# SYSTRAN/faster-whisper

Hardware: AMD Instinct MI355X
Metric: audio-sec/sec (RTF) large-v3 fp16 beam=5 batch=16 (higher is better)
Workload: dtype f16

## Files before the change

### faster_whisper_amd/_lib.py

```python
import ctypes as C
import os

import numpy as np

_HERE = os.path.dirname(os.path.abspath(__file__))
LIB_PATH = os.environ.get("FWAMD_LIB") or os.path.join(_HERE, "libfwamd.so")

FW_OK = 0
FW_EINVAL = -1
FW_ENODEV = -2
FW_ENOMEM = -3
FW_ERUNTIME = -4
FW_ENOSPC = -5

COMPUTE_FLOAT16 = 0
COMPUTE_INT8_FLOAT16 = 1
FW_DT_F32 = 0
FW_DT_F16 = 1
FW_MAX_ALIGN_HEADS = 64


class FwConfig(C.Structure):
    _fields_ = [
        ("n_mels", C.c_int32), ("n_audio_ctx", C.c_int32), ("d_model", C.c_int32), ("n_heads", C.c_int32),
        ("n_enc_layers", C.c_int32), ("n_dec_layers", C.c_int32), ("n_vocab", C.c_int32),
        ("n_text_ctx", C.c_int32), ("is_multilingual", C.c_int32),
        ("tok_eot", C.c_int32), ("tok_sot", C.c_int32), ("tok_lang_begin", C.c_int32), ("n_langs", C.c_int32),
        ("tok_translate", C.c_int32), ("tok_transcribe", C.c_int32), ("tok_sot_lm", C.c_int32),
        ("tok_sot_prev", C.c_int32), ("tok_no_speech", C.c_int32), ("tok_no_timestamps", C.c_int32),
        ("tok_timestamp_begin", C.c_int32),
        ("n_suppress_begin", C.c_int32), ("suppress_begin", C.c_int32 * 8),
        ("n_align_heads", C.c_int32), ("align_heads", C.c_int32 * (2 * FW_MAX_ALIGN_HEADS)),
    ]


class FwWeight(C.Structure):
    _fields_ = [("name", C.c_char_p), ("data", C.c_void_p), ("dtype", C.c_int32), ("ndim", C.c_int32),
                ("dims", C.c_int64 * 4)]


class FwGenOpts(C.Structure):
    _fields_ = [
        ("beam_size", C.c_int32), ("patience", C.c_float), ("num_hypotheses", C.c_int32),
        ("length_penalty", C.c_float), ("repetition_penalty", C.c_float), ("no_repeat_ngram_size", C.c_int32),
        ("max_length", C.c_int32), ("return_scores", C.c_int32), ("return_no_speech_prob", C.c_int32),
        ("max_initial_timestamp_index", C.c_int32), ("suppress_blank", C.c_int32),
        ("suppress_tokens", C.POINTER(C.c_int32)), ("n_suppress_tokens", C.c_int32),
        ("sampling_topk", C.c_int32), ("sampling_temperature", C.c_float), ("seed", C.c_uint64),
        ("min_new_tokens", C.c_int32),
    ]


class FwVadWeights(C.Structure):
    _fields_ = [
        ("stft_basis", C.c_void_p), ("conv_w", C.c_void_p * 4), ("conv_b", C.c_void_p * 4),
        ("lstm_w", C.c_void_p), ("lstm_r", C.c_void_p), ("lstm_b", C.c_void_p), ("dec_w", C.c_void_p),
        ("dec_b", C.c_float),
    ]


SYMBOLS = [
    "fw_last_error", "fw_abi_version", "fw_device_count",
    "fw_model_create", "fw_model_free", "fw_model_info", "fw_model_blob", "fw_model_create_from_blob_dev",
    "fw_model_set_decode_batch", "fw_model_decode_batch", "fw_model_join_decoder", "fw_model_decode_stats",
    "fw_model_set_merge_wait", "fw_model_set_decode_lanes", "fw_model_run_capacity", "fw_dec_big_min_rows", "fw_dec_big_min_rows_of", "fw_test_knob",
    "fw_test_idle_lead_chunks",
    "fw_pack_blob_size", "fw_pack_blob_copy", "fw_pack_blob_free",
    "fw_logmel", "fw_logmel_full",
    "fw_encode", "fw_encode_pcm", "fw_encode_pcm_dev", "fw_tensor_shape", "fw_tensor_to_host",
    "fw_tensor_from_host", "fw_tensor_free",
    "fw_generate", "fw_detect_language", "fw_align",
    "fw_prof_enable", "fw_prof_reset", "fw_prof_count", "fw_prof_name", "fw_prof_get", "fw_synchronize",
    "fw_dev_alloc", "fw_dev_free", "fw_dev_upload",
    "fw_test_gemm", "fw_test_layernorm", "fw_test_attention", "fw_test_dec_linear", "fw_test_dec_logits", "fw_test_logits_rules",
    "fw_test_dec_self_attn", "fw_test_dec_cross_attn", "fw_test_dec_cross_probs", "fw_test_dec_softmax_pick", "fw_bench_gemm", "fw_bench_dec_linear", "fw_bench_attention",
    "fw_bench_gemm_epi", "fw_bench_dec_linear_epi",
    "fw_test_gemm_ex", "fw_test_cross_kv_frag_index", "fw_test_quant_rows", "fw_test_layernorm_frag",
    "fw_vad_create", "fw_vad_forward", "fw_vad_free", "fw_vad_forward_dev", "fw_vad_forward_audio_dev",
    "fw_flac_info", "fw_flac_decode",
    "fw_resample_filter", "fw_resample_dev", "fw_bench_resample",
]

_lib = None


class FwError(RuntimeError):
    pass


def load():
    global _lib
    if _lib is not None:
        return _lib
    if not os.path.exists(LIB_PATH):
        raise FwError(
            f"{LIB_PATH} not found: build it with `python -c 'import __graft_entry__ as g; g.build()'` "
            "(hipcc --offload-arch=gfx950). faster_whisper_amd has no CPU fallback.")
    lib = C.CDLL(LIB_PATH)
    vp, i32, i64, f32p = C.c_void_p, C.c_int32, C.c_int64, C.POINTER(C.c_float)
    i32p, i64p = C.POINTER(C.c_int32), C.POINTER(C.c_int64)
    lib.fw_last_error.restype = C.c_char_p
    lib.fw_abi_version.restype = i32
    lib.fw_device_count.restype = i32
    lib.fw_model_create.argtypes = [C.POINTER(FwConfig), C.POINTER(FwWeight), i32, i32, i32, i32, i32, C.POINTER(vp)]
    lib.fw_model_free.argtypes = [vp]
    lib.fw_model_free.restype = None
    lib.fw_model_info.argtypes = [vp, C.POINTER(FwConfig), i32p, i32p, i32p, i32p]
    lib.fw_model_blob.argtypes = [vp, C.POINTER(vp), i64p]
    lib.fw_model_create_from_blob_dev.argtypes = [C.POINTER(FwConfig), vp, i64, i32, i32, i32, i32, C.POINTER(vp)]
    lib.fw_model_set_decode_batch.argtypes = [vp, i32]
    lib.fw_model_decode_batch.argtypes = [vp]
    lib.fw_model_decode_batch.restype = i32
    lib.fw_model_run_capacity.argtypes = [vp]
    lib.fw_model_run_capacity.restype = i32
    lib.fw_dec_big_min_rows.restype = i32
    if hasattr(lib, "fw_dec_big_min_rows_of"):
        lib.fw_dec_big_min_rows_of.restype = i32
        lib.fw_dec_big_min_rows_of.argtypes = [i32, i32]
    if hasattr(lib, "fw_flac_info"):
        lib.fw_flac_info.argtypes = [vp, i64, i32p, i32p, i32p, i64p]
        lib.fw_flac_decode.argtypes = [vp, i64, vp, i64, i64p, i32p]
    if hasattr(lib, "fw_test_knob"):
        lib.fw_test_knob.argtypes = [i32, i32]
    if hasattr(lib, "fw_test_idle_lead_chunks"):
        lib.fw_test_idle_lead_chunks.argtypes = [i64, i32, i32, i64, i32]
        lib.fw_test_idle_lead_chunks.restype = i64
    lib.fw_model_join_decoder.argtypes = [vp, vp]
    lib.fw_model_set_merge_wait.argtypes = [vp, i32, i32]
    lib.fw_model_set_decode_lanes.argtypes = [vp, i32]
    lib.fw_model_decode_stats.argtypes = [vp, i64p, i64p, i64p, i32p]
    lib.fw_pack_blob_size.argtypes = [C.POINTER(FwConfig), C.POINTER(FwWeight), i32, i32, i64p, C.POINTER(vp)]
    lib.fw_pack_blob_copy.argtypes = [vp, vp, i64]
    lib.fw_pack_blob_free.argtypes = [vp]
    lib.fw_pack_blob_free.restype = None
    lib.fw_logmel.argtypes = [vp, vp, i64p, i32, vp, i32p]
    lib.fw_logmel_full.argtypes = [vp, vp, i64, vp, i64]
    lib.fw_encode.argtypes = [vp, vp, i32, C.POINTER(vp)]
    lib.fw_encode_pcm.argtypes = [vp, vp, i64p, i32, C.POINTER(vp)]
    lib.fw_encode_pcm_dev.argtypes = [vp, vp, i64p, i32, C.POINTER(vp)]
    lib.fw_tensor_shape.argtypes = [vp, i32p, i32p, i32p]
    lib.fw_tensor_to_host.argtypes = [vp, vp, vp]
    lib.fw_tensor_from_host.argtypes = [vp, vp, i32, C.POINTER(vp)]
    lib.fw_tensor_free.argtypes = [vp]
    lib.fw_tensor_free.restype = None
    lib.fw_generate.argtypes = [vp, vp, i32p, i32p, i32, C.POINTER(FwGenOpts), i32p, i32p, f32p, f32p]
    lib.fw_detect_language.argtypes = [vp, vp, i32, i32p, f32p]
    lib.fw_align.argtypes = [vp, vp, i32p, i32, i32p, i32p, i32p, i32, i32, i32, i32p, i32p, f32p]
    lib.fw_prof_enable.argtypes = [vp, i32]
    lib.fw_prof_enable.restype = None
    lib.fw_prof_reset.argtypes = [vp]
    lib.fw_prof_reset.restype = None
    lib.fw_prof_count.restype = i32
    lib.fw_prof_name.argtypes = [i32]
    lib.fw_prof_name.restype = C.c_char_p
    lib.fw_prof_get.argtypes = [vp, i32, C.POINTER(C.c_double), i64p, C.POINTER(C.c_double), C.POINTER(C.c_double)]
    lib.fw_synchronize.argtypes = [vp]
    lib.fw_dev_alloc.argtypes = [vp, i64, C.POINTER(vp)]
    lib.fw_dev_free.argtypes = [vp, vp]
    lib.fw_dev_upload.argtypes = [vp, vp, vp, i64]
    lib.fw_test_gemm.argtypes = [vp, vp, vp, vp, vp, i32, i32, i32, i32, i32, vp]
    lib.fw_test_dec_linear.argtypes = [vp, vp, vp, vp, vp, vp, vp, i32, i32, i32, i32, i32, vp, vp]
    lib.fw_test_dec_logits.argtypes = [vp, vp, i32, vp]
    lib.fw_test_logits_rules.argtypes = [vp, vp, i32, vp, i32, vp, C.POINTER(FwGenOpts), i32, vp, vp]
    if hasattr(lib, "fw_test_dec_self_attn"):
        lib.fw_test_dec_self_attn.argtypes = [vp, vp, vp, vp, vp, i32, i32, i32, i32, i32, i32, i32, i32, i32, i32, i32, vp]
        lib.fw_test_dec_cross_attn.argtypes = [vp, vp, vp, vp, i32, i32, i32, i32, i32, i32, vp, vp, i32, C.c_float, vp]
        lib.fw_test_dec_cross_probs.argtypes = [vp, vp, vp, i32, i32, i32, vp, i32, i32, i32, i32, vp]
        lib.fw_test_dec_softmax_pick.argtypes = [vp, vp, i32, i32, i32, vp, i32, vp]
    lib.fw_bench_attention.argtypes = [vp, i32, i32, i32, i32, i32, f32p]
    lib.fw_bench_gemm.argtypes = [vp, i32, i32, i32, i32, i32, i32, i32, i32, f32p]
    lib.fw_bench_dec_linear.argtypes = [vp, i32, i32, i32, i32, i32, i32, f32p]
    if hasattr(lib, "fw_bench_gemm_epi"):
        lib.fw_bench_gemm_epi.argtypes = [vp, i32, i32, i32, i32, i32, i32, i32, i32, i32, i32, i32, f32p]
        lib.fw_bench_dec_linear_epi.argtypes = [vp, i32, i32, i32, i32, i32, i32, i32, i32, i32, f32p]
    lib.fw_test_layernorm.argtypes = [vp, vp, vp, vp, i32, i32, vp]
    lib.fw_test_attention.argtypes = [vp, vp, vp, vp, i32, i32, i32, vp]
    if hasattr(lib, "fw_test_gemm_ex"):
        lib.fw_test_gemm_ex.argtypes = [vp, vp, i64, i64, i64, vp, vp, vp, i64, i64, i64, vp, i64, i64, i64, i64, i64,
                                        i32, i32, i32, i32, i32, i32, i32, i32, i32, vp, vp]
        lib.fw_test_cross_kv_frag_index.argtypes = [i32, i32, i32, vp]
        lib.fw_test_quant_rows.argtypes = [vp, vp, i32, i32, i64, vp, vp, i32, vp, vp]
        lib.fw_test_layernorm_frag.argtypes = [vp, vp, vp, vp, i32, i32, i32, vp]
    lib.fw_vad_create.argtypes = [C.POINTER(FwVadWeights), C.POINTER(vp)]
    lib.fw_vad_forward.argtypes = [vp, vp, i64, i32, vp, vp, vp]
    lib.fw_vad_free.argtypes = [vp]
    lib.fw_vad_forward_dev.argtypes = [vp, i32, vp, i64, vp, vp, vp]
    if hasattr(lib, "fw_vad_forward_audio_dev"):
        lib.fw_vad_forward_audio_dev.argtypes = [vp, i32, vp, i64, vp, vp, vp]
    lib.fw_vad_free.restype = None
    if hasattr(lib, "fw_resample_dev"):
        f64 = C.c_double
        lib.fw_resample_filter.argtypes = [i32, i32, i32, f64, vp, i64p, i32p, i32p]
        lib.fw_resample_dev.argtypes = [i32, vp, i64, i32, i32, i32, f64, i32, vp, i64]
        lib.fw_bench_resample.argtypes = [i32, vp, i64, i32, i32, i32, f64, i32, i32, f32p]
    _lib = lib
    return lib


def check(rc: int):
    if rc == FW_OK:
        return
    msg = load().fw_last_error().decode("utf-8", "replace")
    if rc in (FW_EINVAL, FW_ENOSPC):
        raise ValueError(msg)
    raise RuntimeError(f"libfwamd error {rc}: {msg}")


def ptr(a: np.ndarray):
    return a.ctypes.data_as(C.c_void_p)


def as_i32p(a: np.ndarray):
    return a.ctypes.data_as(C.POINTER(C.c_int32))


def as_i64p(a: np.ndarray):
    return a.ctypes.data_as(C.POINTER(C.c_int64))


def as_f32p(a: np.ndarray):
    return a.ctypes.data_as(C.POINTER(C.c_float))
```

### faster_whisper_amd/csrc/dec_kernels.h

```cpp
#pragma once
#include "common.h"

namespace fwd {

constexpr int FIN_CAP = 48;

struct GenDev {
  int B, K, R;
  int P;
  int budget;
  int max_fin;
  int V, n_text_ctx;
  int with_ts, suppress_blank, min_new, mits, ngram;
  float rep_pen, lp_pow;
  int eot, no_ts, ts_begin;
  int n_sup_begin, sup_begin[8];
  int sample;
  float inv_temp;
  unsigned seed_lo, seed_hi;
  int kv_div;
  int ctx, cache_rows;
};

void launch_embed(hipStream_t st, const int* tok, const half_t* emb, const half_t* pos_emb, half_t* x, half_t* xfrag,
                  int rows, int d,
                  const int* d_step, int pos_fixed, int P, int blk_n = 0);
bool self_attn_block_ok(int n_ctx, int cache_ctx, int d, int R_total);
void launch_self_attn(hipStream_t st, const half_t* qkv, int d, half_t* kc, half_t* vc, int n_ctx, int cache_ctx, int H,
                      const uint8_t* kvidx2, int Kbeam, int kmul, half_t* out, int rows, const int* d_step,
                      int pos_fixed, int P, int R_total, int frag, int blk_n = 0);
void set_self_attn_form(int form);
void set_cross_attn_regs(int cap);
int kernel_forms_epoch();
void bump_kernel_forms_epoch();
void launch_cross_attn(hipStream_t st, const half_t* qx, int d, const half_t* ck, const half_t* cvt, int T, int kvp,
                       int kmul, half_t* out, int B, int H, const int* done, int kv_div, int frag, const int* slot_map);
int dec_big_min_rows();
int dec_big_min_rows_of(int role, int compute_type);
int launch_dec_gemm_frag(hipStream_t st, const half_t* xf, const half_t* Wf, const half_t* bias, const float* s1,
                         const float* cf, const half_t* res, int ldr, half_t* out, int ldo, half_t* out_frag, int R,
                         int N, int K, int act);
int launch_dec_gemm_skinny(hipStream_t st, const half_t* xf, const half_t* Wf, const half_t* bias, const float* s1,
                           const float* cf, const half_t* res, int ldr, half_t* out, int ldo, half_t* out_frag, int R,
                           int N, int K, int act);
int launch_dec_gemm_skinny_tiles(hipStream_t st, int tiles, const half_t* xf, const half_t* Wf, const half_t* bias,
                                 const float* s1, const float* cf, const half_t* res, int ldr, half_t* out, int ldo,
                                 half_t* out_frag, int R, int N, int K, int act);
int launch_dec_gemm_big(hipStream_t st, int cfg, const half_t* xf, const half_t* Wf, const half_t* bias, const float* s1,
                        const float* cf, const half_t* res, int ldr, half_t* out, int ldo, half_t* out_frag, int R,
                        int N, int K, int act);
int launch_dec_gemm_frag_variant(hipStream_t st, int variant, bool lnf, const half_t* xf, const half_t* Wf,
                                 const half_t* bias, const float* s1, const float* cf, half_t* out, int R, int N,
                                 int K);
int launch_dec_gemm_frag_i8(hipStream_t st, const int8_t* xq, const float* x_scale, const int8_t* Wq,
                            const float* w_scale, const half_t* bias, const half_t* res, int ldr, half_t* out, int ldo,
                            int R, int N, int K, int act);
int launch_dec_logits(hipStream_t st, bool i8, const void* xf, const float* x_scale, const void* Wf,
                      const float* w_scale, const float* s1, const float* cf, float* out, int ldo, int R, int N, int K);
void launch_nospeech(hipStream_t st, const float* logits, int V, int row_mul, int no_speech_id, float* out, int B);
#define LP_SUP_WORDS 896
void launch_logits_process(hipStream_t st, const GenDev& gp, float* logits, const unsigned long long* sup_bits,
                           const int* hist2, const float* cum2, const int* d_step, const int* done, float* cand_val,
                           int* cand_tok);
void launch_beam_update(hipStream_t st, const GenDev& gp, const float* cand_val, const int* cand_tok, int* hist2,
                        float* cum2, uint8_t* kvidx2, int* cur_tok, const int* d_step, int* done, int* n_done,
                        int* n_fin, int* fin_tok, int* fin_len, float* fin_score, float* fin_cum);
void launch_step_advance(hipStream_t st, int* d_step);
void launch_token_prob(hipStream_t st, const float* logits, int V, const int* target, float* out, int out_stride,
                       int out_off, int rows, int row_mul = 1);
void launch_cross_probs(hipStream_t st, const half_t* qx, int d, const half_t* ck, int T, int kvp, const int* heads,
                        int n_layer_heads, int n_sel, float* probs, int n_tok, int tok_idx, int B, int blk_n = 0);

}
```

### faster_whisper_amd/csrc/dec_kernels.hip

```cpp
#include "common.h"
#include "dec_kernels.h"
#include <stdlib.h>
#include <atomic>
#include <type_traits>

namespace fwd {
static std::atomic<int> g_self_attn_form{0};
static std::atomic<int> g_forms_epoch{0};
static std::atomic<int> g_cross_regs{0};
}

__device__ __forceinline__ size_t frag_off(int row, int k, int KS) {
  return ((size_t)((row >> 4) * KS + (k >> 5)) * 64 + ((k >> 3) & 3) * 16 + (row & 15)) * 8 + (k & 7);
}

__global__ void dec_embed_kernel(const int* __restrict__ tok, const half_t* __restrict__ emb,
                                 const half_t* __restrict__ pos_emb, half_t* __restrict__ x,
                                 half_t* __restrict__ xfrag, int d, const int* __restrict__ d_step, int pos_fixed,
                                 int P, int blk_n) {
  const int r = blockIdx.x;
  const int pos = blk_n > 0 ? pos_fixed + r % blk_n : (pos_fixed >= 0 ? pos_fixed : P - 1 + *d_step);
  const half2_t* e = reinterpret_cast<const half2_t*>(emb + (size_t)tok[r] * d);
  const half2_t* pe = reinterpret_cast<const half2_t*>(pos_emb + (size_t)pos * d);
  half2_t* xo = reinterpret_cast<half2_t*>(x + (size_t)r * d);
  for (int i = threadIdx.x; i < d / 2; i += blockDim.x) {
    const half2_t a = e[i], b = pe[i];
    half2_t o;
    o[0] = (half_t)((float)a[0] + (float)b[0]);
    o[1] = (half_t)((float)a[1] + (float)b[1]);
    xo[i] = o;
    if (xfrag) *reinterpret_cast<half2_t*>(xfrag + frag_off(r, 2 * i, d >> 5)) = o;
  }
}

static __device__ __forceinline__ void dec_ln_stats(float sa, float sb, int K, float& mu, float& rstd) {
#pragma clang fp contract(off)
  const float kf = (float)K;
  mu = sa / kf;
  const float ex2 = sb / kf;
  const float var = ex2 - mu * mu;
  rstd = rsqrtf(fmaxf(var, 0.f) + 1e-5f);
}
struct DecColConsts { floatx4 a4, c4; half4_t b4; };
template <bool LNF>
static __device__ __forceinline__ DecColConsts dec_col_consts(const float* __restrict__ s1, const float* __restrict__ cf,
                                                              const half_t* __restrict__ bias, int n) {
  DecColConsts k;
  k.a4 = floatx4{0.f, 0.f, 0.f, 0.f}; k.c4 = k.a4;
  k.b4 = half4_t{(half_t)0.f, (half_t)0.f, (half_t)0.f, (half_t)0.f};
  if (LNF) {
    k.a4 = *reinterpret_cast<const floatx4*>(s1 + n);
    k.c4 = *reinterpret_cast<const floatx4*>(cf + n);
  } else if (bias) {
    k.b4 = *reinterpret_cast<const half4_t*>(bias + n);
  }
  return k;
}
template <bool LNF>
static __device__ __forceinline__ half4_t dec_epilogue4(const floatx4 v, float mu, float rstd, const floatx4 a4,
                                                        const floatx4 c4, const half4_t b4, bool bias, bool has_res,
                                                        half4_t r4, int act) {
#pragma clang fp contract(off)
  half4_t o;
#pragma unroll
  for (int e = 0; e < 4; ++e) {
    float tv = v[e];
    if (LNF) {
      const float t = tv - mu * a4[e];
      tv = rstd * t + c4[e];
    } else if (bias) {
      tv = tv + (float)b4[e];
    }
    if (act == 1) {
      const float er = erff(tv * 0.70710678118654752440f);
      tv = (0.5f * tv) * (1.0f + er);
    }
    if (has_res) tv = tv + (float)r4[e];
    o[e] = (half_t)tv;
  }
  return o;
}

static __device__ __forceinline__ half4_t dec_epilogue4_i8(const int (&v)[4], float sx, const float* __restrict__ w_scale,
                                                           const half_t* __restrict__ bias, const half_t* __restrict__ res,
                                                           int ldr, int row, int n, int act) {
#pragma clang fp contract(off)
  const floatx4 w4 = *reinterpret_cast<const floatx4*>(w_scale + n);
  half4_t b4 = {(half_t)0.f, (half_t)0.f, (half_t)0.f, (half_t)0.f}, r4 = b4;
  if (bias) b4 = *reinterpret_cast<const half4_t*>(bias + n);
  if (res) r4 = *reinterpret_cast<const half4_t*>(res + (size_t)row * ldr + n);
  half4_t o;
#pragma unroll
  for (int e = 0; e < 4; ++e) {
    float tv = ((float)v[e] * sx) * w4[e];
    if (bias) tv = tv + (float)b4[e];
    if (act == 1) {
      const float er = erff(tv * 0.70710678118654752440f);
      tv = (0.5f * tv) * (1.0f + er);
    }
    if (res) tv = tv + (float)r4[e];
    o[e] = (half_t)tv;
  }
  return o;
}

template <int WAVES, bool LNF, int RT, int NT, int CH_ = 0>
__global__ __launch_bounds__(WAVES * 64) void dec_gemm_frag_kernel(
    const half_t* __restrict__ xf, const half_t* __restrict__ Wf, const half_t* __restrict__ bias,
    const float* __restrict__ s1, const float* __restrict__ cf, const half_t* __restrict__ res, int ldr,
    half_t* __restrict__ out, int ldo, half_t* __restrict__ out_frag, int R, int N, int K, int act) {
  __shared__ float red[WAVES][RT * NT][64][4];
  __shared__ float red_s[WAVES][RT][16][2];
  constexpr int CH = CH_ ? CH_ : 20 / (RT + NT);
  const int lane = threadIdx.x & 63;
  const int wave = __builtin_amdgcn_readfirstlane(threadIdx.x >> 6);
  const int i = lane & 15, g = lane >> 4;
  const int n_rt = (R + 15) >> 4;
  const int ct0 = blockIdx.x * NT, rt0 = blockIdx.y * RT;
  const int KS = K >> 5;
  const int per = (KS + WAVES - 1) / WAVES;
  const int ks0 = wave * per;
  int nks = KS - ks0;
  if (nks > per) nks = per;
  floatx4 acc[RT][NT];
  float rs[RT], rq[RT];
#pragma unroll
  for (int a = 0; a < RT; ++a) {
    rs[a] = 0.f; rq[a] = 0.f;
#pragma unroll
    for (int b = 0; b < NT; ++b) acc[a][b] = floatx4{0, 0, 0, 0};
  }
  constexpr bool CONSTS_EARLY = !(LNF && RT * NT > 1);
  half4_t resv[(RT * NT + WAVES - 1) / WAVES];
  DecColConsts colk[(RT * NT + WAVES - 1) / WAVES];
#pragma unroll
  for (int q = 0; q < (RT * NT + WAVES - 1) / WAVES; ++q) {
    resv[q] = half4_t{(half_t)0.f, (half_t)0.f, (half_t)0.f, (half_t)0.f};
    colk[q] = DecColConsts{floatx4{0.f, 0.f, 0.f, 0.f}, floatx4{0.f, 0.f, 0.f, 0.f}, resv[q]};
  }
#pragma unroll
  for (int a = 0; a < RT; ++a) {
#pragma unroll
    for (int b = 0; b < NT; ++b) {
      if ((a * NT + b) % WAVES != wave) continue;
      int row = (rt0 + a) * 16 + i, n = (ct0 + b) * 16 + 4 * g;
      if (row > R - 1) row = R - 1;
      if (n > N - 4) n = N - 4;
      if (CONSTS_EARLY) colk[(a * NT + b) / WAVES] = dec_col_consts<LNF>(s1, cf, bias, n);
      if (res) resv[(a * NT + b) / WAVES] = *reinterpret_cast<const half4_t*>(res + (size_t)row * ldr + n);
    }
  }
  if (nks > 0) {
    const half8_t* wp[NT];
    const half8_t* xp[RT];
#pragma unroll
    for (int b = 0; b < NT; ++b) {
      int ct = ct0 + b;
      if (ct > (N >> 4) - 1) ct = (N >> 4) - 1;
      wp[b] = reinterpret_cast<const half8_t*>(Wf) + ((size_t)ct * KS + ks0) * 64 + lane;
    }
#pragma unroll
    for (int a = 0; a < RT; ++a) {
      int rt = rt0 + a;
      if (rt > n_rt - 1) rt = n_rt - 1;
      xp[a] = reinterpret_cast<const half8_t*>(xf) + ((size_t)rt * KS + ks0) * 64 + lane;
    }
    for (int c = 0; c < nks; c += CH) {
      half8_t wv[NT][CH], xv[RT][CH];
#pragma unroll
      for (int j = 0; j < CH; ++j) {
        const int jj = (c + j < nks) ? c + j : nks - 1;
#pragma unroll
        for (int b = 0; b < NT; ++b) wv[b][j] = wp[b][(size_t)jj * 64];
#pragma unroll
        for (int a = 0; a < RT; ++a) xv[a][j] = xp[a][(size_t)jj * 64];
      }
#pragma unroll
      for (int j = 0; j < CH; ++j) {
        if (c + j < nks) {
#pragma unroll
          for (int a = 0; a < RT; ++a) {
#pragma unroll
            for (int b = 0; b < NT; ++b)
              acc[a][b] = __builtin_amdgcn_mfma_f32_16x16x32_f16(wv[b][j], xv[a][j], acc[a][b], 0, 0, 0);
            if (LNF) {
              const half2_t one2 = {(half_t)1.f, (half_t)1.f};
#pragma unroll
              for (int e = 0; e < 4; ++e) {
                const half2_t h2 = {xv[a][j][2 * e], xv[a][j][2 * e + 1]};
                rs[a] = __builtin_amdgcn_fdot2(h2, one2, rs[a], false);
                rq[a] = __builtin_amdgcn_fdot2(h2, h2, rq[a], false);
              }
            }
          }
        }
      }
    }
  }
  if (!CONSTS_EARLY) {
#pragma unroll
    for (int a = 0; a < RT; ++a) {
#pragma unroll
      for (int b = 0; b < NT; ++b) {
        if ((a * NT + b) % WAVES != wave) continue;
        int n = (ct0 + b) * 16 + 4 * g;
        if (n > N - 4) n = N - 4;
        colk[(a * NT + b) / WAVES] = dec_col_consts<LNF>(s1, cf, bias, n);
      }
    }
  }
#pragma unroll
  for (int a = 0; a < RT; ++a) {
    if (LNF) {
      float sa = rs[a], sb = rq[a];
      sa += __shfl_xor(sa, 16, 64); sa += __shfl_xor(sa, 32, 64);
      sb += __shfl_xor(sb, 16, 64); sb += __shfl_xor(sb, 32, 64);
      if (g == 0) { red_s[wave][a][i][0] = sa; red_s[wave][a][i][1] = sb; }
    }
#pragma unroll
    for (int b = 0; b < NT; ++b)
#pragma unroll
      for (int e = 0; e < 4; ++e) red[wave][a * NT + b][lane][e] = acc[a][b][e];
  }
  __syncthreads();
#pragma unroll
  for (int a = 0; a < RT; ++a) {
#pragma unroll
    for (int b = 0; b < NT; ++b) {
      if ((a * NT + b) % WAVES != wave) continue;
      const int row = (rt0 + a) * 16 + i;
      if (row >= R) continue;
      float v[4] = {0.f, 0.f, 0.f, 0.f};
#pragma unroll
      for (int w = 0; w < WAVES; ++w)
#pragma unroll
        for (int e = 0; e < 4; ++e) v[e] += red[w][a * NT + b][lane][e];
      float mu = 0.f, rstd = 1.f;
      if (LNF) {
        float sa = 0.f, sb = 0.f;
#pragma unroll
        for (int w = 0; w < WAVES; ++w) { sa += red_s[w][a][i][0]; sb += red_s[w][a][i][1]; }
        dec_ln_stats(sa, sb, K, mu, rstd);
      }
      const int n = (ct0 + b) * 16 + 4 * g;
      if (n >= N) continue;
      const floatx4 v4 = {v[0], v[1], v[2], v[3]};
      const half4_t r4 = resv[(a * NT + b) / WAVES];
      const DecColConsts& ck = colk[(a * NT + b) / WAVES];
      const half4_t o = dec_epilogue4<LNF>(v4, mu, rstd, ck.a4, ck.c4, ck.b4, bias != nullptr, res != nullptr, r4, act);
      if (out) *reinterpret_cast<half4_t*>(out + (size_t)row * ldo + n) = o;
      if (out_frag) *reinterpret_cast<half4_t*>(out_frag + frag_off(row, n, N >> 5)) = o;
    }
  }
}

#ifndef DGB_TL
#define DGB_TL(slot) do {} while (0)
#define DGB_TL_DECL
#endif
template <int N_>
static __device__ __forceinline__ void wait_vmcnt() {
  asm volatile("s_waitcnt vmcnt(%0)" ::"n"(N_) : "memory");
}
#define DGB_BARRIER()                      \
  do {                                     \
    asm volatile("" ::: "memory");         \
    __builtin_amdgcn_s_barrier();          \
    asm volatile("" ::: "memory");         \
  } while (0)

#define DGB_BARRIER_LDS() __syncthreads()

template <bool LNF, int S, int WM, int WN, int FB, int KC, int NST>
__global__ __launch_bounds__(WM * WN * 64, 2) void dec_gemm_big_kernel(
    const half_t* __restrict__ xf, const half_t* __restrict__ Wf, const half_t* __restrict__ bias,
    const float* __restrict__ s1, const float* __restrict__ cf, const half_t* __restrict__ res, int ldr,
    half_t* __restrict__ out, int ldo, half_t* __restrict__ out_frag, int R, int N, int K, int act, int nNt) {
  constexpr int NW = WM * WN;
  DGB_TL_DECL;
  constexpr int PX = 4 * WM, PW = FB * WN, PCS = PX + PW;
  static_assert((PCS * KC) % NW == 0, "pieces of a stage must divide over the waves");
  static_assert(FB == 2 || FB == 4, "column tiles per wave");
  constexpr int PPW = PCS * KC / NW;
  constexpr int STAGE_BYTES = PCS * KC * 1024;
  static_assert(NST >= 3 && NST <= 6, "ring depth");
  constexpr int DGB_EP_STRIDE = FB * 32 + 16;
  static_assert(NST * STAGE_BYTES >= NW * 64 * DGB_EP_STRIDE, "the epilogue stages one 64-row patch per wave through the ring");
  extern __shared__ __attribute__((aligned(16))) char dgb_smem[];
  const int lane = threadIdx.x & 63;
  const int wave = __builtin_amdgcn_readfirstlane(threadIdx.x >> 6);
  const int i = lane & 15, g = lane >> 4;
  const int wm = wave / WN, wn = wave % WN;
  const int bid = xcd_remap(blockIdx.x, gridDim.x);
  const int nMt = gridDim.x / nNt;
  const int nt = bid / nMt, mt = bid - nt * nMt;
  const int rt0 = mt * PX, ct0 = nt * PW;
  const int n_rt = (R + 15) >> 4;
  const int KS = K >> 5;
  const int per = KS / S;
  const int nch = KS / KC;
  const int ch_per_slice = per / KC;

  unsigned soff[PPW];
  const char* sbase[PPW];
#pragma unroll
  for (int q = 0; q < PPW; ++q) {
    const int p = wave * PPW + q;
    const int t = p / KC, ks = p % KC;
    if (t < PX) {
      int rt = rt0 + t;
      if (rt > n_rt - 1) rt = n_rt - 1;
      sbase[q] = reinterpret_cast<const char*>(xf);
      soff[q] = (unsigned)((((size_t)rt * KS + ks) * 64 + lane) * 16);
    } else {
      int ct = ct0 + t - PX;
      if (ct > (N >> 4) - 1) ct = (N >> 4) - 1;
      sbase[q] = reinterpret_cast<const char*>(Wf);
      soff[q] = (unsigned)((((size_t)ct * KS + ks) * 64 + lane) * 16);
    }
  }
  auto issue = [&](int c, int slot) {
    char* dst = dgb_smem + slot * STAGE_BYTES + wave * PPW * 1024;
    const unsigned koff = (unsigned)c * (KC * 1024);
#pragma unroll
    for (int q = 0; q < PPW; ++q)
      __builtin_amdgcn_global_load_lds((const __attribute__((address_space(1))) void*)(sbase[q] + (size_t)(soff[q] + koff)),
                                       (__attribute__((address_space(3))) void*)(dst + q * 1024), 16, 0, 0);
  };

  static_assert(!LNF || WN == 2, "the LayerNorm statistics are shared by the TWO waves of a row block");
  floatx4 acc[4][FB], tot[4][FB];
  float rs[2] = {0.f, 0.f}, rq[2] = {0.f, 0.f}, sal[2] = {0.f, 0.f}, sbl[2] = {0.f, 0.f};
  float sa[4], sb[4];
#pragma unroll
  for (int a = 0; a < 4; ++a) {
    sa[a] = 0.f; sb[a] = 0.f;
#pragma unroll
    for (int b = 0; b < FB; ++b) { acc[a][b] = floatx4{0, 0, 0, 0}; tot[a][b] = floatx4{0, 0, 0, 0}; }
  }

  half8_t xv[KC][4], wv[KC][FB];
  auto fetch = [&](int slot) {
    const char* st = dgb_smem + slot * STAGE_BYTES;
#pragma unroll
    for (int ks = 0; ks < KC; ++ks) {
#pragma unroll
      for (int a = 0; a < 4; ++a)
        xv[ks][a] = *reinterpret_cast<const half8_t*>(st + (((wm * 4 + a) * KC + ks) * 64 + lane) * 16);
#pragma unroll
      for (int b = 0; b < FB; ++b)
        wv[ks][b] = *reinterpret_cast<const half8_t*>(st + (((PX + wn * FB + b) * KC + ks) * 64 + lane) * 16);
    }
    __builtin_amdgcn_sched_barrier(0);
  };
  auto mma = [&]() {
    __builtin_amdgcn_sched_barrier(0);
    DGB_TL(4);
#pragma unroll
    for (int ks = 0; ks < KC; ++ks) {
      if (LNF) {
        const half2_t one2 = {(half_t)1.f, (half_t)1.f};
        const half8_t xs0 = wn ? xv[ks][2] : xv[ks][0], xs1 = wn ? xv[ks][3] : xv[ks][1];
#pragma unroll
        for (int e = 0; e < 4; ++e) {
          const half2_t h0 = {xs0[2 * e], xs0[2 * e + 1]}, h1 = {xs1[2 * e], xs1[2 * e + 1]};
          rs[0] = __builtin_amdgcn_fdot2(h0, one2, rs[0], false);
          rq[0] = __builtin_amdgcn_fdot2(h0, h0, rq[0], false);
          rs[1] = __builtin_amdgcn_fdot2(h1, one2, rs[1], false);
          rq[1] = __builtin_amdgcn_fdot2(h1, h1, rq[1], false);
        }
      }
#pragma unroll
      for (int b = 0; b < FB; ++b) {
#pragma unroll
        for (int a = 0; a < 4; ++a)
          acc[a][b] = __builtin_amdgcn_mfma_f32_16x16x32_f16(wv[ks][b], xv[ks][a], acc[a][b], 0, 0, 0);
      }
    }
  };
  auto compute = [&](int slot) { fetch(slot); mma(); };
  auto slice_end = [&]() {
    if (LNF) {
#pragma unroll
      for (int aa = 0; aa < 2; ++aa) {
        float pa = rs[aa], pb = rq[aa];
        pa += __shfl_xor(pa, 16, 64); pa += __shfl_xor(pa, 32, 64);
        pb += __shfl_xor(pb, 16, 64); pb += __shfl_xor(pb, 32, 64);
        sal[aa] += pa; sbl[aa] += pb;
        rs[aa] = 0.f; rq[aa] = 0.f;
      }
    }
#pragma unroll
    for (int a = 0; a < 4; ++a) {
#pragma unroll
      for (int b = 0; b < FB; ++b) {
#pragma unroll
        for (int e = 0; e < 4; ++e) tot[a][b][e] += acc[a][b][e];
        acc[a][b] = floatx4{0, 0, 0, 0};
      }
    }
  };

#pragma unroll
  for (int c0 = 0; c0 < NST - 1; ++c0) issue(c0, c0);
  int slot = 0, fill = NST - 1;
  int to_slice = ch_per_slice;
  const int n_steady = nch - (NST - 1);
  for (int c = 0; c < n_steady; ++c) {
    DGB_TL(0);
    wait_vmcnt<(NST - 2) * PPW>();
    DGB_TL(1);
    DGB_BARRIER();
    DGB_TL(2);
    fetch(slot);
    DGB_TL(3);
    issue(c + NST - 1, fill);
    mma();
    DGB_TL(5);
    if (--to_slice == 0) { to_slice = ch_per_slice; slice_end(); }
    fill = slot;
    slot = (slot + 1 == NST) ? 0 : slot + 1;
  }
  wait_vmcnt<0>();
  const int row0 = (rt0 + wm * 4) * 16;
  const int col0 = (ct0 + wn * FB) * 16;
  constexpr int CPR = FB * 2;
  constexpr int RPI = 64 / CPR;
  const int cr = lane / CPR, cc = lane % CPR;
  constexpr int NSEG = 64 / RPI;
  constexpr int RES_EARLY = (LNF && NW == 8 && FB == 4) ? 2 : NSEG;
  DecColConsts colk[FB];
  intx4 resv[NSEG];
  auto load_res = [&](int j0, int j1) {
    if (!res) return;
#pragma unroll
    for (int j = 0; j < NSEG; ++j) {
      if (j < j0 || j >= j1) continue;
      int row = row0 + j * RPI + cr, n = col0 + cc * 8;
      if (row > R - 1) row = R - 1;
      if (n > N - 8) n = N - 8;
      resv[j] = *reinterpret_cast<const intx4*>(res + (size_t)row * ldr + n);
    }
  };
#pragma unroll
  for (int b = 0; b < FB; ++b) {
    int n = col0 + b * 16 + 4 * g;
    if (n > N - 4) n = N - 4;
    colk[b] = dec_col_consts<LNF>(s1, cf, bias, n);
  }
  load_res(0, RES_EARLY);
#pragma unroll 1
  for (int c = n_steady; c < nch; ++c) {
    DGB_BARRIER();
    compute(slot);
    if (--to_slice == 0) { to_slice = ch_per_slice; slice_end(); }
    slot = (slot + 1 == NST) ? 0 : slot + 1;
  }
  load_res(RES_EARLY, NSEG);
  DGB_BARRIER();

  if (LNF) {
    float* xch = reinterpret_cast<float*>(dgb_smem);
    if (g == 0) {
#pragma unroll
      for (int aa = 0; aa < 2; ++aa) {
        xch[((wave * 2 + aa) * 16 + i) * 2] = sal[aa];
        xch[((wave * 2 + aa) * 16 + i) * 2 + 1] = sbl[aa];
      }
    }
    DGB_BARRIER_LDS();
#pragma unroll
    for (int a = 0; a < 4; ++a) {
      const int owner = (wave & ~1) | (a >> 1);
      sa[a] = xch[((owner * 2 + (a & 1)) * 16 + i) * 2];
      sb[a] = xch[((owner * 2 + (a & 1)) * 16 + i) * 2 + 1];
    }
    DGB_BARRIER_LDS();
  }
  char* ep = dgb_smem + wave * (64 * DGB_EP_STRIDE);
  if (res) {
#pragma unroll
    for (int j = 0; j < 64 / RPI; ++j) {
      const int r = j * RPI + cr;
      *reinterpret_cast<intx4*>(ep + r * DGB_EP_STRIDE + cc * 16) = resv[j];
    }
  }
#pragma unroll
  for (int a = 0; a < 4; ++a) {
    float mu = 0.f, rstd = 1.f;
    if (LNF) dec_ln_stats(sa[a], sb[a], K, mu, rstd);
#pragma unroll
    for (int b = 0; b < FB; ++b) {
      char* cell = ep + (a * 16 + i) * DGB_EP_STRIDE + (b * 16 + 4 * g) * 2;
      half4_t r4 = {(half_t)0.f, (half_t)0.f, (half_t)0.f, (half_t)0.f};
      if (res) r4 = *reinterpret_cast<const half4_t*>(cell);
      const half4_t o = dec_epilogue4<LNF>(tot[a][b], mu, rstd, colk[b].a4, colk[b].c4, colk[b].b4, bias != nullptr,
                                           res != nullptr, r4, act);
      *reinterpret_cast<half4_t*>(cell) = o;
    }
  }
  if (out) {
#pragma unroll
    for (int j = 0; j < 64 / RPI; ++j) {
      const int r = j * RPI + cr;
      const int row = row0 + r, n = col0 + cc * 8;
      const intx4 v = *reinterpret_cast<const intx4*>(ep + r * DGB_EP_STRIDE + cc * 16);
      if (row < R && n < N) *reinterpret_cast<intx4*>(out + (size_t)row * ldo + n) = v;
    }
  }
  if (out_frag) {
    const int KSo = N >> 5;
#pragma unroll
    for (int a = 0; a < 4; ++a) {
#pragma unroll
      for (int kb = 0; kb < FB / 2; ++kb) {
        const int row = row0 + a * 16 + i, n = col0 + kb * 32 + g * 8;
        const intx4 v = *reinterpret_cast<const intx4*>(ep + (a * 16 + i) * DGB_EP_STRIDE + (kb * 32 + g * 8) * 2);
        if (row < R && n < N)
          *reinterpret_cast<intx4*>(out_frag + ((size_t)((row >> 4) * KSo + (n >> 5)) * 64 + lane) * 8) = v;
      }
    }
  }
}

template <int WAVES, int RT, int NT, int CH_ = 0>
__global__ __launch_bounds__(WAVES * 64) void dec_gemm_frag_i8_kernel(
    const int8_t* __restrict__ xq, const float* __restrict__ x_scale, const int8_t* __restrict__ Wq,
    const float* __restrict__ w_scale, const half_t* __restrict__ bias, const half_t* __restrict__ res, int ldr,
    half_t* __restrict__ out, int ldo, int R, int N, int K, int act) {
  __shared__ int red[WAVES][RT * NT][64][4];
  constexpr int CH = CH_ ? CH_ : 20 / (RT + NT);
  const int lane = threadIdx.x & 63;
  const int wave = __builtin_amdgcn_readfirstlane(threadIdx.x >> 6);
  const int i = lane & 15, g = lane >> 4;
  const int ct0 = blockIdx.x * NT, rt0 = blockIdx.y * RT;
  const int n_rt = (R + 15) >> 4;
  const int KS = K >> 6;
  const int per = (KS + WAVES - 1) / WAVES;
  const int ks0 = wave * per;
  int nks = KS - ks0;
  if (nks > per) nks = per;
// ... 351 lines not shown
  }
}

template <int U, bool PIPE, int MAXT, bool PB = false>
__global__ __launch_bounds__(MAXT) void dec_self_attn2_kernel(const half_t* __restrict__ qkv, int d, half_t* __restrict__ kc,
                                                             half_t* __restrict__ vc, int n_ctx, int cache_ctx,
                                                             int H, const uint8_t* __restrict__ kvidx2, int Kbeam, int kmul,
                                                             half_t* __restrict__ out, const int* __restrict__ d_step,
                                                             int pos_fixed, int P, int R_total, int frag) {
  extern __shared__ float sa_smem[];
  constexpr int NB = 4 * U;
  const int lane = threadIdx.x & 63;
  const int wave = __builtin_amdgcn_readfirstlane(threadIdx.x >> 6);
  float* sp = sa_smem + (size_t)wave * 2 * n_ctx;
  int* ssrc = reinterpret_cast<int*>(sp + n_ctx);
  const int h = blockIdx.x, c = blockIdx.y;
  const int r = c * kmul + wave, kb = PB ? 0 : wave;
  const int step = PB ? 0 : *d_step;
  const int pos = PB ? pos_fixed + wave : (pos_fixed >= 0 ? pos_fixed : P - 1 + step);
  const int slot = c * Kbeam + kb;
  const int cur = (pos_fixed >= 0) ? 0 : (step & 1);
  const uint8_t* kvidx = kvidx2 + ((size_t)cur * R_total + slot) * n_ctx;
  const half_t* qr = qkv + (size_t)r * 3 * d + h * 64;
  const size_t head_stride = (size_t)cache_ctx * 64;
  const size_t slot_stride = (size_t)H * head_stride;
  const int pg = lane >> 3, cc = lane & 7;
  for (int p4 = 4 * lane; p4 < pos; p4 += 256) {
    const unsigned w = PB ? 0u : *reinterpret_cast<const unsigned*>(kvidx + p4);
    intx4 s4;
    s4[0] = c * Kbeam + (int)(w & 0xffu); s4[1] = c * Kbeam + (int)((w >> 8) & 0xffu);
    s4[2] = c * Kbeam + (int)((w >> 16) & 0xffu); s4[3] = c * Kbeam + (int)(w >> 24);
    *reinterpret_cast<intx4*>(ssrc + p4) = s4;
  }
  const half8_t q8 = *reinterpret_cast<const half8_t*>(qr + cc * 8);
  const half8_t kn8 = *reinterpret_cast<const half8_t*>(qr + d + cc * 8);
  const half8_t vn8 = *reinterpret_cast<const half8_t*>(qr + 2 * d + cc * 8);
  float q[8];
#pragma unroll
  for (int e = 0; e < 8; ++e) q[e] = (float)q8[e] * 0.125f;
  if (pg == 0) {
    *reinterpret_cast<half8_t*>(kc + slot * slot_stride + h * head_stride + (size_t)pos * 64 + cc * 8) = kn8;
    *reinterpret_cast<half8_t*>(vc + slot * slot_stride + h * head_stride + (size_t)pos * 64 + cc * 8) = vn8;
  }
  auto dot8 = [&](const half8_t& k) {
    float sacc = 0.f;
#pragma unroll
    for (int e = 0; e < 8; ++e) sacc = __builtin_fmaf(q[e], (float)k[e], sacc);
    return sum8_dpp(sacc);
  };
  const float s_new = dot8(kn8);
  float mx = s_new;
  __builtin_amdgcn_wave_barrier();
  const char* kbase = reinterpret_cast<const char*>(kc + h * head_stride);
  const char* vbase = reinterpret_cast<const char*>(vc + h * head_stride);
  const unsigned slot_bytes = (unsigned)(slot_stride * sizeof(half_t));
  struct Batch { half8_t row[NB]; };
  auto fetch = [&](Batch& b, const char* base, int p0, const half_t* sib) {
#pragma unroll
    for (int j = 0; j < NB; ++j) {
      const int p = p0 + 8 * j + pg;
      const int pc = p < pos ? p : pos - 1;
      const unsigned off = (unsigned)ssrc[pc] * slot_bytes + (unsigned)(pc * 128 + cc * 16);
      if (PB && pc >= pos_fixed)
        b.row[j] = *reinterpret_cast<const half8_t*>(sib + (size_t)(pc - pos_fixed) * 3 * d + cc * 8);
      else
        b.row[j] = *reinterpret_cast<const half8_t*>(base + off);
    }
  };
  const half_t* ksib = qkv + (size_t)c * kmul * 3 * d + d + h * 64;
  const half_t* vsib = ksib + d;
  auto score = [&](const Batch& b, int p0) {
#pragma unroll
    for (int j = 0; j < NB; ++j) {
      const int p = p0 + 8 * j + pg;
      const float sc = dot8(b.row[j]);
      if (p < pos) {
        if (cc == 0) sp[p] = sc;
        mx = fmaxf(mx, sc);
      }
    }
  };
  Batch b0, b1;
  if (pos > 0) {
    fetch(b0, kbase, 0, ksib);
    for (int p0 = 0; p0 < pos; p0 += 16 * NB) {
      if (PIPE) {
        fetch(b1, kbase, p0 + 8 * NB, ksib);
        score(b0, p0);
        fetch(b0, kbase, p0 + 16 * NB, ksib);
        score(b1, p0 + 8 * NB);
      } else {
        score(b0, p0);
        if (p0 + 8 * NB < pos) {
          fetch(b0, kbase, p0 + 8 * NB, ksib);
          score(b0, p0 + 8 * NB);
          if (p0 + 16 * NB < pos) fetch(b0, kbase, p0 + 16 * NB, ksib);
        }
      }
    }
    fetch(b0, vbase, 0, vsib);
  }
  mx = wave_max_v(mx);
  __builtin_amdgcn_wave_barrier();
  float sum = 0.f;
  for (int p = lane; p < pos; p += 64) {
    const float e = __expf(sp[p] - mx);
    sp[p] = e;
    sum += e;
  }
  const float e_new = __expf(s_new - mx);
  sum = wave_sum_v(sum) + e_new;
  __builtin_amdgcn_wave_barrier();
  float acc[8];
#pragma unroll
  for (int e = 0; e < 8; ++e) acc[e] = 0.f;
  auto accum = [&](const Batch& b, int p0) {
#pragma unroll
    for (int j = 0; j < NB; ++j) {
      const int p = p0 + 8 * j + pg;
      if (p < pos) {
        const float w = sp[p];
#pragma unroll
        for (int e = 0; e < 8; ++e) acc[e] = __builtin_fmaf(w, (float)b.row[j][e], acc[e]);
      }
    }
  };
  for (int p0 = 0; p0 < pos; p0 += 16 * NB) {
    if (PIPE) {
      fetch(b1, vbase, p0 + 8 * NB, vsib);
      accum(b0, p0);
      fetch(b0, vbase, p0 + 16 * NB, vsib);
      accum(b1, p0 + 8 * NB);
    } else {
      accum(b0, p0);
      if (p0 + 8 * NB < pos) {
        fetch(b0, vbase, p0 + 8 * NB, vsib);
        accum(b0, p0 + 8 * NB);
        if (p0 + 16 * NB < pos) fetch(b0, vbase, p0 + 16 * NB, vsib);
      }
    }
  }
#pragma unroll
  for (int e = 0; e < 8; ++e) acc[e] = sum_x8_x16_x32_v(acc[e]);
  if (pg == 0) {
    const float inv = 1.f / sum;
    half8_t o;
#pragma unroll
    for (int e = 0; e < 8; ++e) o[e] = (half_t)((acc[e] + e_new * (float)vn8[e]) * inv);
    half_t* dst = frag ? out + frag_off(r, h * 64 + cc * 8, d >> 5) : out + (size_t)r * d + h * 64 + cc * 8;
    *reinterpret_cast<half8_t*>(dst) = o;
  }
}

template <int CA_WAVES, bool NTL, int MINW = 1>
__global__ __launch_bounds__(CA_WAVES * 64, MINW) void dec_cross_attn_kernel(const half_t* __restrict__ qx, int d,
                                                             const half_t* __restrict__ ck,
                                                             const half_t* __restrict__ cvt, int T, int kvp,
                                                             int kmul, half_t* __restrict__ out,
                                                             const int* __restrict__ done, int kv_div, int frag,
                                                             const int* __restrict__ slot_map) {
  __shared__ float sm[CA_WAVES][16], sl[CA_WAVES][16];
  __shared__ float so[CA_WAVES][16][65];
  const int h = blockIdx.x, c = blockIdx.y;
  if (done && done[c]) return;
  const int tid = threadIdx.x, lane = tid & 63, wave = tid >> 6;
  const int j = lane & 15, g = lane >> 4;
  const int ce = slot_map[c / kv_div];
  const half_t* kbase = ck + ((size_t)ce * (d >> 6) + h) * kvp * 64 + lane * 8;
  const half_t* vbase = cvt + ((size_t)ce * (d >> 6) + h) * kvp * 64 + lane * 8;
  half8_t qf[2];
  {
    if (j < kmul) {
      const half_t* qp = qx + (size_t)(c * kmul + j) * d + h * 64 + g * 8;
#pragma unroll
      for (int s = 0; s < 2; ++s) {
        half8_t v = *reinterpret_cast<const half8_t*>(qp + s * 32);
#pragma unroll
        for (int e = 0; e < 8; ++e) v[e] = v[e] * (half_t)0.125f;
        qf[s] = v;
      }
    } else {
      qf[0] = half8_t{0, 0, 0, 0, 0, 0, 0, 0};
      qf[1] = qf[0];
    }
  }
  floatx4 o[4];
#pragma unroll
  for (int dt = 0; dt < 4; ++dt) o[dt] = floatx4{0, 0, 0, 0};
  float m_run = -1.0e30f, l_run = 0.f;
  const float LOG2E = 1.4426950408889634f;
  const int ngroups = (T + 31) >> 5;
  auto load_kv = [&](int gi, half8_t (&kf)[4], half8_t (&vf)[4]) {
    const half_t* kp = kbase + (size_t)gi * 2048;
    const half_t* vp = vbase + (size_t)gi * 2048;
#pragma unroll
    for (int q = 0; q < 4; ++q)
      kf[q] = NTL ? __builtin_nontemporal_load(reinterpret_cast<const half8_t*>(kp + q * 512))
                  : *reinterpret_cast<const half8_t*>(kp + q * 512);
#pragma unroll
    for (int dt = 0; dt < 4; ++dt)
      vf[dt] = NTL ? __builtin_nontemporal_load(reinterpret_cast<const half8_t*>(vp + dt * 512))
                   : *reinterpret_cast<const half8_t*>(vp + dt * 512);
  };
  half8_t kcur[4], vcur[4], knxt[4], vnxt[4];
  if (wave < ngroups) load_kv(wave, kcur, vcur);
  for (int gi = wave; gi < ngroups; gi += CA_WAVES) {
    const int base = gi * 32;
    const bool has_next = (gi + CA_WAVES) < ngroups;
    if (has_next) load_kv(gi + CA_WAVES, knxt, vnxt);
    floatx4 s0 = {0, 0, 0, 0}, s1 = {0, 0, 0, 0};
    s0 = __builtin_amdgcn_mfma_f32_16x16x32_f16(kcur[0], qf[0], s0, 0, 0, 0);
    s0 = __builtin_amdgcn_mfma_f32_16x16x32_f16(kcur[1], qf[1], s0, 0, 0, 0);
    s1 = __builtin_amdgcn_mfma_f32_16x16x32_f16(kcur[2], qf[0], s1, 0, 0, 0);
    s1 = __builtin_amdgcn_mfma_f32_16x16x32_f16(kcur[3], qf[1], s1, 0, 0, 0);
    float sc[8];
    float mx = -1.0e30f;
#pragma unroll
    for (int e = 0; e < 8; ++e) {
      float v = (e < 4 ? s0[e] : s1[e - 4]) * LOG2E;
      if (base + 8 * g + e >= T) v = -1.0e30f;
      sc[e] = v;
      mx = fmaxf(mx, v);
    }
    mx = pair16_max(mx);
    mx = pair32_max(mx);
    const float m_new = fmaxf(m_run, mx);
    const float alpha = __builtin_amdgcn_exp2f(m_run - m_new);
    m_run = m_new;
    half8_t pf;
    float psum = 0.f;
#pragma unroll
    for (int e = 0; e < 8; ++e) {
      const float pv = __builtin_amdgcn_exp2f(sc[e] - m_new);
      psum += pv;
      pf[e] = (half_t)pv;
    }
    l_run = l_run * alpha + psum;
#pragma unroll
    for (int dt = 0; dt < 4; ++dt) {
#pragma unroll
      for (int e = 0; e < 4; ++e) o[dt][e] *= alpha;
      o[dt] = __builtin_amdgcn_mfma_f32_16x16x32_f16(vcur[dt], pf, o[dt], 0, 0, 0);
    }
    if (has_next) {
#pragma unroll
      for (int q = 0; q < 4; ++q) { kcur[q] = knxt[q]; vcur[q] = vnxt[q]; }
    }
  }
  l_run = pair16_sum(l_run);
  l_run = pair32_sum(l_run);
  if (g == 0) { sm[wave][j] = m_run; sl[wave][j] = l_run; }
#pragma unroll
  for (int dt = 0; dt < 4; ++dt)
#pragma unroll
    for (int e = 0; e < 4; ++e) so[wave][j][dt * 16 + 4 * g + e] = o[dt][e];
  __syncthreads();
  for (int idx = tid; idx < kmul * 64; idx += CA_WAVES * 64) {
    const int qq = idx >> 6, dh = idx & 63;
    float M = sm[0][qq];
#pragma unroll
    for (int w = 1; w < CA_WAVES; ++w) M = fmaxf(M, sm[w][qq]);
    float Lsum = 0.f, O = 0.f;
#pragma unroll
    for (int w = 0; w < CA_WAVES; ++w) {
      const float f = __builtin_amdgcn_exp2f(sm[w][qq] - M);
      Lsum += sl[w][qq] * f;
      O += so[w][qq][dh] * f;
    }
    const int orow = c * kmul + qq;
    half_t* dst = frag ? out + frag_off(orow, h * 64 + dh, d >> 5) : out + (size_t)orow * d + h * 64 + dh;
    *dst = (half_t)(O / Lsum);
  }
}

__global__ __launch_bounds__(1024) void dec_nospeech_kernel(const float* __restrict__ logits, int V, int row_mul,
                                                            int no_speech_id, float* __restrict__ out) {
  __shared__ float red[32];
  const int b = blockIdx.x;
  const float* lg = logits + (size_t)b * row_mul * V;
  float mx = -3.0e38f;
  for (int v = threadIdx.x; v < V; v += blockDim.x) mx = fmaxf(mx, lg[v]);
  mx = wave_max(mx);
  if ((threadIdx.x & 63) == 0) red[threadIdx.x >> 6] = mx;
  __syncthreads();
  float m2 = -3.0e38f;
  for (int i = 0; i < (int)(blockDim.x >> 6); ++i) m2 = fmaxf(m2, red[i]);
  __syncthreads();
  float s = 0.f;
  for (int v = threadIdx.x; v < V; v += blockDim.x) s += __expf(lg[v] - m2);
  s = wave_sum(s);
  if ((threadIdx.x & 63) == 0) red[threadIdx.x >> 6] = s;
  __syncthreads();
  if (threadIdx.x == 0) {
    float tot = 0.f;
    for (int i = 0; i < (int)(blockDim.x >> 6); ++i) tot += red[i];
    out[b] = __expf(lg[no_speech_id] - m2) / tot;
  }
}

#define LP_THREADS 1024
#define LP_WAVES (LP_THREADS / 64)
#define LP_NV 56
static __device__ __forceinline__ float gumbel_noise(unsigned seed_lo, unsigned seed_hi, unsigned row, unsigned step,
                                                     unsigned v) {
  unsigned h = seed_lo ^ (row * 0x9E3779B9u) ^ (step * 0x85EBCA6Bu) ^ (v * 0xC2B2AE35u) ^ (seed_hi * 0x27D4EB2Fu);
  h ^= h >> 16; h *= 0x85EBCA6Bu; h ^= h >> 13; h *= 0xC2B2AE35u; h ^= h >> 16;
  const float u = ((float)(h >> 9) + 0.5f) * (1.0f / 8388608.0f);
  return -logf(-logf(u));
}

template <bool SMP, int TXI>
__global__ __launch_bounds__(LP_THREADS) void dec_logits_process_kernel(fwd::GenDev gp, float* __restrict__ logits,
                                                                        const unsigned long long* __restrict__ sup_bits,
                                                                        const int* __restrict__ hist2,
                                                                        const float* __restrict__ cum2,
                                                                        const int* __restrict__ d_step,
                                                                        const int* __restrict__ done,
                                                                        float* __restrict__ cand_val,
                                                                        int* __restrict__ cand_tok) {
  __shared__ float red_mt[LP_WAVES], red_ms[LP_WAVES], red_st[LP_WAVES], red_ss[LP_WAVES];
  __shared__ float bkey_s[2][LP_WAVES];
  __shared__ int btok_s[2][LP_WAVES];
  __shared__ int sh_last_ts;
  const int r = blockIdx.x;
  const int c = r / gp.K;
  if (done[c]) return;
  const int tid = threadIdx.x;
  const int lane = tid & 63;
  const int wv = __builtin_amdgcn_readfirstlane(tid >> 6);
  const int step = *d_step;
  const int cur = step & 1;
  const int n = step;
  const int* hist = hist2 + ((size_t)cur * gp.R + r) * gp.n_text_ctx;
  float* lg = logits + (size_t)r * gp.V;
  const int V = gp.V, tb = gp.ts_begin;
  const float NEG = -INFINITY;
  const int NONE = 0x7fffffff;

  if (gp.rep_pen != 1.0f && n > 0) {
    for (int i = tid; i < n; i += LP_THREADS) {
      const int t = hist[i];
      bool first = true;
      for (int q = 0; q < i; ++q)
        if (hist[q] == t) { first = false; break; }
      if (first) {
        const float v = lg[t];
        lg[t] = v < 0.f ? v * gp.rep_pen : v / gp.rep_pen;
      }
    }
    __syncthreads();
  }
  if (gp.ngram > 0 && n + 1 >= gp.ngram) {
    const int k = gp.ngram;
    for (int s = tid; s + k <= n; s += LP_THREADS) {
      bool match = true;
      for (int q = 0; q < k - 1; ++q)
        if (hist[s + q] != hist[n - (k - 1) + q]) { match = false; break; }
      if (match) lg[hist[s + k - 1]] = NEG;
// ... 445 lines not shown
static int dec_big_cfg_for(int R, int N, int K) {
  const DecBigRule* r = DEC_BIG_RULES[dec_linear_role(N, K)];
  if (R >= r[1].rows) return r[1].cfg;
  if (R >= r[0].rows) return r[0].cfg;
  return -1;
}
#define DEC_BIG_MIN_ROWS_I8 1024
int dec_big_min_rows_of(int role, int compute_type) {
  if (compute_type == 1) return DEC_BIG_MIN_ROWS_I8;
  if (role >= 0 && role < 4) return DEC_BIG_RULES[role][0].rows;
  int lo = DEC_BIG_RULES[0][0].rows;
  for (int k = 1; k < 4; ++k) lo = DEC_BIG_RULES[k][0].rows < lo ? DEC_BIG_RULES[k][0].rows : lo;
  return lo;
}

static bool skinny_one_tile(int R, int N) { return R <= 16 || (R <= 96 && N <= 1280); }

int launch_dec_gemm_frag(hipStream_t st, const half_t* xf, const half_t* Wf, const half_t* bias, const float* s1,
                         const float* cf, const half_t* res, int ldr, half_t* out, int ldo, half_t* out_frag, int R,
                         int N, int K, int act) {
  const int cfg = dec_big_cfg_for(R, N, K);
  if (cfg >= 0 &&
      launch_dec_gemm_big(st, cfg, xf, Wf, bias, s1, cf, res, ldr, out, ldo, out_frag, R, N, K, act) == 0)
    return 0;
  return launch_dec_gemm_skinny(st, xf, Wf, bias, s1, cf, res, ldr, out, ldo, out_frag, R, N, K, act);
}

int dec_big_min_rows() { return dec_big_min_rows_of(-1, 0); }

int launch_dec_gemm_skinny(hipStream_t st, const half_t* xf, const half_t* Wf, const half_t* bias, const float* s1,
                           const float* cf, const half_t* res, int ldr, half_t* out, int ldo, half_t* out_frag, int R,
                           int N, int K, int act) {
  if (K % 32 != 0 || N % 32 != 0 || R < 1) return -1;
  const int waves = K >= 2560 ? 8 : 4;
  const bool one_tile = skinny_one_tile(R, N);
  if (one_tile) {
    if (s1) frag_go<true, 1, 1, 10>(st, waves, xf, Wf, bias, s1, cf, res, ldr, out, ldo, out_frag, R, N, K, act);
    else frag_go<false, 1, 1, 10>(st, waves, xf, Wf, bias, s1, cf, res, ldr, out, ldo, out_frag, R, N, K, act);
    return 0;
  }
  if (s1) frag_go<true, 2, 2>(st, waves, xf, Wf, bias, s1, cf, res, ldr, out, ldo, out_frag, R, N, K, act);
  else frag_go<false, 2, 2>(st, waves, xf, Wf, bias, s1, cf, res, ldr, out, ldo, out_frag, R, N, K, act);
  return 0;
}

int launch_dec_gemm_skinny_tiles(hipStream_t st, int tiles, const half_t* xf, const half_t* Wf, const half_t* bias,
                                 const float* s1, const float* cf, const half_t* res, int ldr, half_t* out, int ldo,
                                 half_t* out_frag, int R, int N, int K, int act) {
  if (K % 32 != 0 || N % 32 != 0 || R < 1) return -1;
  const int waves = K >= 2560 ? 8 : 4;
  if (tiles == 1) {
    if (s1) frag_go<true, 1, 1, 10>(st, waves, xf, Wf, bias, s1, cf, res, ldr, out, ldo, out_frag, R, N, K, act);
    else frag_go<false, 1, 1, 10>(st, waves, xf, Wf, bias, s1, cf, res, ldr, out, ldo, out_frag, R, N, K, act);
  } else if (tiles == 2) {
    if (s1) frag_go<true, 2, 2>(st, waves, xf, Wf, bias, s1, cf, res, ldr, out, ldo, out_frag, R, N, K, act);
    else frag_go<false, 2, 2>(st, waves, xf, Wf, bias, s1, cf, res, ldr, out, ldo, out_frag, R, N, K, act);
  } else {
    return -1;
  }
  return 0;
}

int launch_dec_gemm_frag_i8(hipStream_t st, const int8_t* xq, const float* x_scale, const int8_t* Wq,
                            const float* w_scale, const half_t* bias, const half_t* res, int ldr, half_t* out, int ldo,
                            int R, int N, int K, int act) {
  if (K % 64 != 0 || N % 32 != 0 || R < 1 || !x_scale || !w_scale) return -1;
  if (R >= DEC_BIG_MIN_ROWS_I8 && N % 64 == 0) {
    const dim3 g4(N / 64, ((R + 15) / 16 + 3) / 4);
    if (K >= 2560)
      dec_gemm_frag_i8_kernel<8, 4, 4, 3><<<g4, 512, 0, st>>>(xq, x_scale, Wq, w_scale, bias, res, ldr, out, ldo, R, N, K, act);
    else
      dec_gemm_frag_i8_kernel<4, 4, 4, 5><<<g4, 256, 0, st>>>(xq, x_scale, Wq, w_scale, bias, res, ldr, out, ldo, R, N, K, act);
    return 0;
  }
  const dim3 grid(N / 32, ((R + 15) / 16 + 1) / 2);
  if (K >= 2560)
    dec_gemm_frag_i8_kernel<8, 2, 2><<<grid, 512, 0, st>>>(xq, x_scale, Wq, w_scale, bias, res, ldr, out, ldo, R, N, K, act);
  else
    dec_gemm_frag_i8_kernel<4, 2, 2><<<grid, 256, 0, st>>>(xq, x_scale, Wq, w_scale, bias, res, ldr, out, ldo, R, N, K, act);
  return 0;
}

template <bool I8, bool LNF, int RT>
static void wave_go(hipStream_t st, const void* xf, const float* x_scale, const void* Wf, const float* w_scale,
                    const float* s1, const float* cf, float* out, int ldo, int R, int N, int K) {
  constexpr int NT = 2, WM = 1, WN = 4;
  const int n_rt = (R + 15) / 16, n_ct = (N + 15) / 16;
  const int n_cg = ((n_ct + NT * WN - 1) / (NT * WN) + 7) & ~7;
  const int n_rg = (n_rt + RT * WM - 1) / (RT * WM);
  dec_gemm_wave_kernel<I8, LNF, true, RT, NT, WM, WN><<<n_cg * n_rg, WM * WN * 64, 0, st>>>(
      xf, x_scale, Wf, w_scale, nullptr, s1, cf, out, ldo, R, N, K, n_rg);
}

int launch_dec_logits(hipStream_t st, bool i8, const void* xf, const float* x_scale, const void* Wf,
                      const float* w_scale, const float* s1, const float* cf, float* out, int ldo, int R, int N, int K) {
  if (K % (i8 ? 64 : 32) != 0 || R < 1) return -1;
  if (i8 ? (!x_scale || !w_scale) : ((s1 == nullptr) != (cf == nullptr))) return -1;
  const int n_rt = (R + 15) / 16;
#define WG(RT)                                                                                   \
  do {                                                                                           \
    if (i8) wave_go<true, false, RT>(st, xf, x_scale, Wf, w_scale, s1, cf, out, ldo, R, N, K);   \
    else if (s1) wave_go<false, true, RT>(st, xf, x_scale, Wf, w_scale, s1, cf, out, ldo, R, N, K); \
    else wave_go<false, false, RT>(st, xf, x_scale, Wf, w_scale, s1, cf, out, ldo, R, N, K);     \
  } while (0)
  if (n_rt == 1) WG(1);
  else if (n_rt == 2) WG(2);
  else if (n_rt == 3) WG(3);
  else if (n_rt == 4) WG(4);
  else WG(5);
#undef WG
  return 0;
}

bool self_attn_block_ok(int n_ctx, int cache_ctx, int d, int R_total) {
  return (n_ctx & 3) == 0 && (size_t)R_total * cache_ctx * d * sizeof(half_t) < ((size_t)1 << 32);
}

void launch_self_attn(hipStream_t st, const half_t* qkv, int d, half_t* kc, half_t* vc, int n_ctx, int cache_ctx, int H,
                      const uint8_t* kvidx2, int Kbeam, int kmul, half_t* out, int rows, const int* d_step,
                      int pos_fixed, int P, int R_total, int frag, int blk_n) {
  if (blk_n > 0) {
    dec_self_attn2_kernel<1, true, 1024, true><<<dim3(H, rows / blk_n), blk_n * 64, (size_t)blk_n * 2 * n_ctx * sizeof(float), st>>>(
        qkv, d, kc, vc, n_ctx, cache_ctx, H, kvidx2, Kbeam, blk_n, out, d_step, pos_fixed, P, R_total, frag);
    return;
  }
  const dim3 grid(H, rows / kmul);
  const size_t lds = (size_t)kmul * 2 * n_ctx * sizeof(float);
  int form = g_self_attn_form.load(std::memory_order_relaxed);
  if ((n_ctx & 3) != 0 || (size_t)R_total * cache_ctx * d * sizeof(half_t) >= ((size_t)1 << 32)) form = 1;
  if (form == 0) form = (kmul <= 8 && (int)(grid.x * grid.y) <= 768) ? 2 : 3;
  if (form == 2 && kmul > 8) form = 3;
#define SA_ARGS qkv, d, kc, vc, n_ctx, cache_ctx, H, kvidx2, Kbeam, kmul, out, d_step, pos_fixed, P, R_total, frag
  if (form == 1) dec_self_attn_kernel<<<grid, kmul * 64, lds, st>>>(SA_ARGS);
  else if (form == 2) dec_self_attn2_kernel<4, false, 512><<<grid, kmul * 64, lds, st>>>(SA_ARGS);
  else dec_self_attn2_kernel<1, true, 1024><<<grid, kmul * 64, lds, st>>>(SA_ARGS);
#undef SA_ARGS
}
void set_self_attn_form(int form) { g_self_attn_form.store(form); g_forms_epoch.fetch_add(1); }
int kernel_forms_epoch() { return g_forms_epoch.load(); }
void bump_kernel_forms_epoch() { g_forms_epoch.fetch_add(1); }

void launch_cross_attn(hipStream_t st, const half_t* qx, int d, const half_t* ck, const half_t* cvt, int T, int kvp,
                       int kmul, half_t* out, int B, int H, const int* done, int kv_div, int frag, const int* slot_map) {
  const int cap = g_cross_regs.load(std::memory_order_relaxed);
  if (cap == 1)
    dec_cross_attn_kernel<8, true, 5><<<dim3(H, B), 512, 0, st>>>(qx, d, ck, cvt, T, kvp, kmul, out, done, kv_div, frag, slot_map);
  else if (cap == 2)
    dec_cross_attn_kernel<8, true, 6><<<dim3(H, B), 512, 0, st>>>(qx, d, ck, cvt, T, kvp, kmul, out, done, kv_div, frag, slot_map);
  else
    dec_cross_attn_kernel<8, true><<<dim3(H, B), 512, 0, st>>>(qx, d, ck, cvt, T, kvp, kmul, out, done, kv_div, frag, slot_map);
}
void set_cross_attn_regs(int cap) { g_cross_regs.store(cap); g_forms_epoch.fetch_add(1); }

void launch_nospeech(hipStream_t st, const float* logits, int V, int row_mul, int no_speech_id, float* out, int B) {
  dec_nospeech_kernel<<<B, 1024, 0, st>>>(logits, V, row_mul, no_speech_id, out);
}

void launch_logits_process(hipStream_t st, const GenDev& gp, float* logits, const unsigned long long* sup_bits,
                           const int* hist2, const float* cum2, const int* d_step, const int* done, float* cand_val,
                           int* cand_tok) {
  const bool wide = gp.ts_begin >= 48 * LP_THREADS;
#define LP_GO(SMP, TXI) \
  dec_logits_process_kernel<SMP, TXI><<<gp.R, LP_THREADS, 0, st>>>(gp, logits, sup_bits, hist2, cum2, d_step, done, cand_val, cand_tok)
  if (gp.sample) { if (wide) LP_GO(true, 48); else LP_GO(true, 0); }
  else { if (wide) LP_GO(false, 48); else LP_GO(false, 0); }
#undef LP_GO
}

void launch_beam_update(hipStream_t st, const GenDev& gp, const float* cand_val, const int* cand_tok, int* hist2,
                        float* cum2, uint8_t* kvidx2, int* cur_tok, const int* d_step, int* done, int* n_done,
                        int* n_fin, int* fin_tok, int* fin_len, float* fin_score, float* fin_cum) {
  dec_beam_update_kernel<<<gp.B, 64, 0, st>>>(gp, cand_val, cand_tok, hist2, cum2, kvidx2, cur_tok, d_step, done,
                                              n_done, n_fin, fin_tok, fin_len, fin_score, fin_cum);
}

void launch_step_advance(hipStream_t st, int* d_step) { dec_step_advance_kernel<<<1, 1, 0, st>>>(d_step); }

void launch_token_prob(hipStream_t st, const float* logits, int V, const int* target, float* out, int out_stride,
                       int out_off, int rows, int row_mul) {
  dec_token_prob_kernel<<<rows, 1024, 0, st>>>(logits, V, target, out, out_stride, out_off, row_mul);
}

void launch_cross_probs(hipStream_t st, const half_t* qx, int d, const half_t* ck, int T, int kvp, const int* heads,
                        int n_layer_heads, int n_sel, float* probs, int n_tok, int tok_idx, int B, int blk_n) {
  const int bn = blk_n > 0 ? blk_n : 1;
  dec_cross_probs_kernel<<<dim3(n_layer_heads, B * bn), 256, 0, st>>>(qx, d, ck, T, kvp, heads, n_sel, probs, n_tok,
                                                                      tok_idx, bn);
}

}
```

### faster_whisper_amd/csrc/decoder.hip

```cpp
#include "engine.h"

#include <math.h>
#include <stdlib.h>
#include <string.h>

#include <algorithm>
#include <atomic>
#include <chrono>
#include <numeric>

#include "dec_kernels.h"
#include "kernels.h"

namespace fw {

using fwd::FIN_CAP;
using fwd::GenDev;

#define DEC_RUN_MAX_ROWS 1600

struct CrossPool {
  half_t *ck = nullptr, *cvt = nullptr;
  int n_blocks = 0, EB = 0, kvp = 0;
  struct Block { uint64_t enc_id = 0; int n = 0; bool busy = false; uint64_t stamp = 0; };
// ... 263 lines not shown
  if (L < 2) return false;
  const int64_t w1 = m->dec[1].ck.w - m->dec[0].ck.w, b1 = m->dec[1].ck.b - m->dec[0].ck.b;
  for (int l = 1; l < L; ++l) {
    if (m->dec[l].ck.w - m->dec[0].ck.w != l * w1 || m->dec[l].cv.w - m->dec[0].cv.w != l * w1) return false;
    if (m->dec[l].ck.b - m->dec[0].ck.b != l * b1 || m->dec[l].cv.b - m->dec[0].cv.b != l * b1) return false;
  }
  *ws = w1; *bs = b1;
  return w1 > 0;
}

static int ensure_cross_kv(Model* m, const Tensor* enc, int blk, bool hit) {
  if (hit) return FW_OK;
  GenWorkspace* g = m->gen;
  CrossPool* pool = pool_of(m);
  const int B = enc->B;
  const int b0 = blk * pool->EB;
  const fw_config& c = m->cfg;
  const int d = c.d_model, T = c.n_audio_ctx;
  const int64_t xs = (int64_t)T * d;
  hipStream_t st = m->dec_stream;
  int rc;
  ProfScope ps(m, PF_CROSS_KV_GEMM, 2.0 * c.n_dec_layers * B * (double)T * d * (2.0 * d), 0, st);
  const bool i8 = m->compute_type == FW_COMPUTE_INT8_FLOAT16;
  const int kvp = pool->kvp;
  const int64_t kvs = (int64_t)d * kvp;
  int64_t ws = 0, bs = 0;
  if (!i8 && cross_kv_layered() && cross_kv_strides(m, &ws, &bs)) {
    const int64_t cls = (int64_t)pool->n_slots() * kvs;
    half_t* kd = pool->ck + (size_t)b0 * kvs;
    half_t* vd = pool->cvt + (size_t)b0 * kvs;
    if ((rc = run_linear_layers(m, m->dec[0].ck, c.n_dec_layers, ws, bs, enc->data, d, xs, kd, d, kvs, cls, T, B, false, kvp, st)))
      return rc;
    if ((rc = run_linear_layers(m, m->dec[0].cv, c.n_dec_layers, ws, bs, enc->data, d, xs, vd, kvp, kvs, cls, T, B, true, kvp, st)))
      return rc;
    std::lock_guard<std::mutex> lk(pool->mu);
    pool->blocks[blk].enc_id = enc->id;
    pool->blocks[blk].n = B;
    return FW_OK;
  }
  for (int l = 0; l < c.n_dec_layers; ++l) {
    const DecLayerW& L = m->dec[l];
    half_t* kd = pool->ck + ((size_t)l * pool->n_slots() + b0) * kvs;
    half_t* vd = pool->cvt + ((size_t)l * pool->n_slots() + b0) * kvs;
    if (i8) {
      if ((rc = run_linear_i8(m, L.ck, l == 0 ? enc->data : nullptr, nullptr, kd, d, kvs, nullptr, 0, 0, T, B, 0,
                              false, kvp, st, g->ekq, g->eks)))
        return rc;
      if ((rc = run_linear_i8(m, L.cv, nullptr, nullptr, vd, kvp, kvs, nullptr, 0, 0, T, B, 0, true, kvp, st, g->ekq,
                              g->eks)))
        return rc;
      continue;
    }
    if ((rc = run_linear(m, L.ck, enc->data, d, xs, kd, d, kvs, nullptr, 0, 0, T, B, 0, false, kvp, st))) return rc;
    if ((rc = run_linear(m, L.cv, enc->data, d, xs, vd, kvp, kvs, nullptr, 0, 0, T, B, 0, true, kvp, st))) return rc;
  }
  {
    std::lock_guard<std::mutex> lk(pool->mu);
    pool->blocks[blk].enc_id = enc->id;
    pool->blocks[blk].n = B;
  }
  return FW_OK;
}

struct StepCfg {
  int rows, kmul;
  int B;
  int pos_fixed;
  int P;
  const int* tok;
  bool need_logits;
  int nospeech_rowmul;
  bool beam_tail;
  const int* done;
  int kv_slot0 = 0;
  int blk_n = 0;
  int nospeech_off = 0;
  const int* sel_heads_dev = nullptr;
  const int* sel_layer_off = nullptr;
  float* probs = nullptr; int n_sel_total = 0, n_tok = 0, tok_idx = 0;
};

#define DG(call)                                                        \
  do {                                                                  \
    if ((call) != 0) {                                                  \
      set_error("decoder gemm: unsupported shape (%s)", #call);        \
      return FW_ERUNTIME;                                               \
    }                                                                   \
  } while (0)

static std::atomic<int> g_pos_blocks{-1};
static bool pos_blocks_on() {
  int v = g_pos_blocks.load(std::memory_order_relaxed);
  if (v < 0) {
    const char* e = getenv("FWAMD_POS_BLOCKS");
    v = (e && atoi(e) == 0) ? 0 : 1;
    g_pos_blocks.store(v);
  }
  return v != 0;
}
void set_pos_blocks(int on) { g_pos_blocks.store(on ? 1 : 0); }
static int pos_block_size(const Model* m, const GenWorkspace* g, const GenDev& gp, int chunks) {
  if (!pos_blocks_on() || chunks < 1) return 1;
  if (!fwd::self_attn_block_ok(g->NT, gp.ctx, m->cfg.d_model, gp.R)) return 1;
  return std::max(1, std::min(16, g->R / chunks));
}

static int run_step(Model* m, const GenDev& gp, const StepCfg& s) {
  GenWorkspace* g = m->gen;
  const fw_config& c = m->cfg;
  const int d = c.d_model, H = c.n_heads, T = c.n_audio_ctx, NT = g->NT;
  CrossPool* pool = pool_of(m);
  const int kvp = pool->kvp;
  hipStream_t st = m->dec_stream;
  const int rows = s.rows;
  const bool i8 = m->compute_type == FW_COMPUTE_INT8_FLOAT16;
  {
    ProfScope ps(m, PF_DEC_MISC, 0, 0, st);
    fwd::launch_embed(st, s.tok, m->tok_emb, m->dec_pos, g->x, i8 ? nullptr : g->x_frag, rows, d, g->d_step,
                      s.pos_fixed, s.P, s.blk_n);
  }
  auto lin_q = [&](const half_t* xin, const LNW* ln, const LinearW& L, const half_t* res, half_t* outp, int act) -> int {
    fwk::launch_quant_rows(st, xin, L.K, ln ? ln->g : nullptr, ln ? ln->b : nullptr, g->xq, g->xs, rows, L.K, 1);
    return fwd::launch_dec_gemm_frag_i8(st, g->xq, g->xs, L.wq, L.wscale, L.b, res, L.N, outp, L.N, rows, L.N, L.K, act);
  };
  auto lin_f = [&](const half_t* xin_frag, const LinearW& L, const half_t* res, half_t* outp, half_t* outp_frag,
                   int act) -> int {
    return fwd::launch_dec_gemm_frag(st, xin_frag, L.w, L.b, L.s1, L.cf, res, L.N, outp, L.N, outp_frag, rows, L.N,
                                     L.K, act);
  };
  const int frag = i8 ? 0 : 1;
  const bool unf = !i8 && m->ln_unfold >= 2;
  auto lin_u = [&](const LNW& ln, const LinearW& L, half_t* outp, half_t* outp_frag, int act) -> int {
    fwk::launch_layernorm(st, g->x, ln.g, ln.b, g->xn_frag, rows, d, 1);
    return fwd::launch_dec_gemm_frag(st, g->xn_frag, L.w, L.b, nullptr, nullptr, nullptr, L.N, outp, L.N, outp_frag, rows,
                                     L.N, L.K, act);
  };
  for (int l = 0; l < c.n_dec_layers; ++l) {
    const DecLayerW& L = m->dec[l];
    half_t* kc = g->sk + (size_t)l * gp.cache_rows * gp.ctx * d;
    half_t* vc = g->sv + (size_t)l * gp.cache_rows * gp.ctx * d;
    const half_t* ck = pool->ck + (size_t)l * pool->n_slots() * d * kvp;
    const half_t* cvt = pool->cvt + (size_t)l * pool->n_slots() * d * kvp;
    {
      ProfScope ps(m, PF_DEC_GEMM_QKV, 2.0 * rows * 3.0 * d * d, 2.0 * 3.0 * d * d, st);
      if (i8) DG(lin_q(g->x, &L.ln1, L.qkv, nullptr, g->qkv, 0));
      else if (unf) DG(lin_u(L.ln1, L.qkv_p, g->qkv, nullptr, 0));
      else DG(lin_f(g->x_frag, L.qkv, nullptr, g->qkv, nullptr, 0));
    }
    {
      ProfScope ps(m, PF_DEC_SELF_ATTN, 0, 0, st);
      fwd::launch_self_attn(st, g->qkv, d, kc, vc, NT, gp.ctx, H, g->kvidx2, gp.K, s.kmul, frag ? g->att_frag : g->att, rows,
                            g->d_step, s.pos_fixed, s.P, gp.R, frag, s.blk_n);
    }
    {
      ProfScope ps(m, PF_DEC_GEMM_DXD, 2.0 * rows * 2.0 * d * d, 2.0 * 2.0 * d * d, st);
      if (i8) {
        DG(lin_q(g->att, nullptr, L.out, g->x, g->x, 0));
        DG(lin_q(g->x, &L.ln2, L.cq, nullptr, g->qc, 0));
      } else {
        DG(lin_f(g->att_frag, L.out, g->x, g->x, g->x_frag, 0));
        if (unf) DG(lin_u(L.ln2, L.cq_p, g->qc, nullptr, 0));
        else DG(lin_f(g->x_frag, L.cq, nullptr, g->qc, nullptr, 0));
      }
    }
    if (s.probs && s.sel_layer_off[l + 1] > s.sel_layer_off[l]) {
      ProfScope ps(m, PF_DEC_MISC, 0, 0, st);
      const int off = s.sel_layer_off[l], n = s.sel_layer_off[l + 1] - off;
      fwd::launch_cross_probs(st, g->qc, d, ck + (size_t)s.kv_slot0 * d * kvp, T, kvp, s.sel_heads_dev + off, n, s.n_sel_total,
                              s.probs + (size_t)off * s.n_tok * T, s.n_tok, s.tok_idx, s.B, s.blk_n);
    }
    {
      ProfScope ps(m, PF_DEC_CROSS_ATTN, 4.0 * rows * (double)T * d, 4.0 * (s.B / gp.kv_div) * (double)T * d, st);
      fwd::launch_cross_attn(st, g->qc, d, ck, cvt, T, kvp, s.kmul, frag ? g->att_frag : g->att, s.B, H, s.done,
                             gp.kv_div, frag, g->slot_map);
    }
    {
      ProfScope ps(m, PF_DEC_GEMM_DXD, 2.0 * rows * 1.0 * d * d, 2.0 * 1.0 * d * d, st);
      if (i8) DG(lin_q(g->att, nullptr, L.cout, g->x, g->x, 0));
      else DG(lin_f(g->att_frag, L.cout, g->x, g->x, g->x_frag, 0));
    }
    {
      ProfScope ps(m, PF_DEC_GEMM_FFN1, 2.0 * rows * 4.0 * d * d, 2.0 * 4.0 * d * d, st);
      if (i8) DG(lin_q(g->x, &L.ln3, L.ffn1, nullptr, g->ffn, 1));
      else if (unf) DG(lin_u(L.ln3, L.ffn1_p, nullptr, g->ffn_frag, 1));
      else DG(lin_f(g->x_frag, L.ffn1, nullptr, nullptr, g->ffn_frag, 1));
    }
    {
      ProfScope ps(m, PF_DEC_GEMM_FFN2, 2.0 * rows * 4.0 * d * d, 2.0 * 4.0 * d * d, st);
      if (i8) DG(lin_q(g->ffn, nullptr, L.ffn2, g->x, g->x, 0));
      else DG(lin_f(g->ffn_frag, L.ffn2, g->x, g->x, g->x_frag, 0));
    }
  }
  if (s.need_logits || s.beam_tail) {
    ProfScope ps(m, PF_DEC_LOGITS, 2.0 * rows * (double)c.n_vocab * d, 2.0 * c.n_vocab * d, st);
    if (i8) {
      fwk::launch_quant_rows(st, g->x, d, m->dec_ln.g, m->dec_ln.b, g->xq, g->xs, rows, d, 1);
      DG(fwd::launch_dec_logits(st, true, g->xq, g->xs, m->logits.wq, m->logits.wscale, nullptr, nullptr, g->logits,
                                c.n_vocab, rows, c.n_vocab, d));
    } else if (m->ln_unfold >= 1) {
      fwk::launch_layernorm(st, g->x, m->dec_ln.g, m->dec_ln.b, g->xn_frag, rows, d, 1);
      DG(fwd::launch_dec_logits(st, false, g->xn_frag, nullptr, m->logits_p.w, nullptr, nullptr, nullptr, g->logits,
                                c.n_vocab, rows, c.n_vocab, d));
    } else {
      DG(fwd::launch_dec_logits(st, false, g->x_frag, nullptr, m->logits.w, nullptr, m->logits.s1, m->logits.cf,
                                g->logits, c.n_vocab, rows, c.n_vocab, d));
    }
  }
  if (s.nospeech_rowmul > 0) {
    ProfScope ps(m, PF_DEC_MISC, 0, 0, st);
    fwd::launch_nospeech(st, g->logits + (size_t)s.nospeech_off * c.n_vocab, c.n_vocab, s.nospeech_rowmul,
                         c.tok_no_speech, g->no_speech, s.B);
  }
  if (s.beam_tail) {
    ProfScope ps(m, PF_DEC_SAMPLE, 0, 8.0 * rows * c.n_vocab, st);
    fwd::launch_logits_process(st, gp, g->logits, g->sup_bits, g->hist2, g->cum2, g->d_step, g->done, g->cand_val,
                               g->cand_tok);
    fwd::launch_beam_update(st, gp, g->cand_val, g->cand_tok, g->hist2, g->cum2, g->kvidx2, g->cur_tok, g->d_step,
                            g->done, g->n_done, g->n_fin, g->fin_tok, g->fin_len, g->fin_score, g->fin_cum);
    fwd::launch_step_advance(st, g->d_step);
  }
  return FW_OK;
}

static int max_new_tokens(int max_length, int P) { return std::max(0, max_length - P); }
static int run_ctx(const fw_config& c, int max_length, int P) {
  const int reach = P + max_new_tokens(std::min(max_length, c.n_text_ctx), P);
  return std::min(c.n_text_ctx, (std::max(reach, 1) + 7) / 8 * 8);
}

static int check_launch(const char* what) {
  hipError_t he = hipGetLastError();
  if (he != hipSuccess) {
    set_error("%s: kernel launch failed: %s", what, hipGetErrorString(he));
    return FW_ERUNTIME;
  }
  return FW_OK;
}

struct GenRequest {
  const Tensor* enc;
  const int32_t* prompts;
  const int32_t* prompt_offsets;
  int B, P;
  const fw_gen_opts* o;
  int32_t* out_ids; int32_t* out_lens; float* out_scores; float* out_no_speech;
  bool sampling;
  int with_ts = 1, sot_pos = -1;
  int rc = FW_OK;
  std::string err;
  bool taken = false;
  bool done = false;
};

static bool mergeable(const GenRequest& a, const GenRequest& b) {
  if (a.sampling || b.sampling) return false;
  const fw_gen_opts &x = *a.o, &y = *b.o;
  if (a.P != b.P || x.beam_size != y.beam_size || x.patience != y.patience || x.num_hypotheses != y.num_hypotheses ||
      x.length_penalty != y.length_penalty || x.repetition_penalty != y.repetition_penalty ||
      x.no_repeat_ngram_size != y.no_repeat_ngram_size || x.max_length != y.max_length ||
      x.max_initial_timestamp_index != y.max_initial_timestamp_index || x.suppress_blank != y.suppress_blank ||
      x.min_new_tokens != y.min_new_tokens || x.n_suppress_tokens != y.n_suppress_tokens)
    return false;
  if (x.n_suppress_tokens && memcmp(x.suppress_tokens, y.suppress_tokens, x.n_suppress_tokens * sizeof(int32_t)))
    return false;
  return a.with_ts == b.with_ts && a.sot_pos == b.sot_pos;
}

static int idle_fill_pct() {
  static const int v = [] {
    const char* e = getenv("FWAMD_IDLE_FILL_PCT");
    const int x = e ? atoi(e) : 100;
    return x < 1 ? 1 : (x > 100 ? 100 : x);
  }();
  return v;
}
static bool idle_balance() {
  static const bool v = [] { const char* e = getenv("FWAMD_IDLE_BALANCE"); return !e || atoi(e) != 0; }();
  return v;
}
int64_t idle_lead_chunks(int64_t queued, int n_queued, int encoding, int64_t want, int max_batch, int lanes) {
  const int64_t per_req = std::max<int64_t>(1, queued / std::max<int64_t>(1, (int64_t)n_queued));
  const int64_t outstanding = queued + (int64_t)std::max(0, encoding) * per_req;
  const int64_t n_runs = std::max<int64_t>(std::max(2, lanes), (outstanding + std::max<int64_t>(1, want) - 1) / std::max<int64_t>(1, want));
  return std::max<int64_t>(max_batch, (outstanding + n_runs - 1) / n_runs);
}
static int64_t planned_self_cap(const Model* dm) {
  const int B = lane_chunks_of(dm);
  const int nts = self_positions(dm, B, dm->decode_self_ctx > 0 ? dm->decode_self_ctx : dm->cfg.n_text_ctx);
  return (int64_t)B * dm->max_beam * nts;
}
static int64_t self_chunk_capacity(Model* dm, const GenRequest& r) {
  const int64_t rows_per_chunk = r.sampling ? std::max(1, r.o->num_hypotheses) : r.o->beam_size;
  return planned_self_cap(dm) / (rows_per_chunk * run_ctx(dm->cfg, r.o->max_length, r.P));
}

static int generate_run(Model* m, const std::vector<GenRequest*>& reqs) {
  int rc = gen_workspace_ensure(m);
  if (rc) return rc;
  GenWorkspace* g = m->gen;
  const fw_config& c = m->cfg;
  const GenRequest& r0 = *reqs[0];
  const fw_gen_opts* o = r0.o;
  const int K = o->beam_size, P = r0.P;
  const bool sampling = r0.sampling;
  const int nh = o->num_hypotheses, ml = o->max_length;
  const int kv_div = sampling ? nh : 1;
  int B = 0;
  for (const GenRequest* r : reqs) B += r->B;
  const int Bx = B * kv_div;
  FW_CHECK_ARG(Bx * K <= g->R && Bx <= g->R && B <= g->B, "decode run of %d chunks x %d rows exceeds the workspace", B,
               kv_div * K);
  const int budget = max_new_tokens(std::min(o->max_length, c.n_text_ctx), P);
  const int ctx = run_ctx(c, o->max_length, P);
  FW_CHECK_ARG((int64_t)Bx * K * ctx <= g->self_cap, "decode run of %d rows x %d positions exceeds the self-attention cache", Bx * K, ctx);
  FW_HIP(hipSetDevice(m->device));
  hipStream_t st = m->dec_stream;
  CrossPool* pool = pool_of(m);
  PoolHold hold{pool, {}, st};
  std::vector<int> slot_host((size_t)Bx);
  {
    std::vector<uint64_t> ids;
    std::vector<int> ns;
    std::vector<char> hit;
    for (const GenRequest* r : reqs) { ids.push_back(r->enc->id); ns.push_back(r->enc->B); }
    FW_CHECK_ARG((int)reqs.size() <= pool->n_blocks, "decode run of %zu calls exceeds the %d blocks of the cross-attention pool",
                 reqs.size(), pool->n_blocks);
    pool_acquire(pool, ids, ns, hold.blk, hit);
// ... 795 lines not shown
```

### faster_whisper_amd/csrc/engine.hip

```cpp
#include "engine.h"

#include <math.h>
#include <stdarg.h>
#include <stdio.h>
#include <stdlib.h>
#include <string.h>

#include <algorithm>

#include "dec_kernels.h"
#include "kernels.h"

namespace fw {

static thread_local char g_err[1024] = "";
void set_error(const char* fmt, ...) {
  va_list ap;
  va_start(ap, fmt);
  vsnprintf(g_err, sizeof(g_err), fmt, ap);
  va_end(ap);
}

int dev_alloc(void** p, size_t bytes) {
  if (bytes == 0) bytes = 256;
// ... 1519 lines not shown
  }
  for (Model* l : fm->impl.xlanes) {
    if (!l) continue;
    prof_collect(l);
    std::lock_guard<std::mutex> lk(l->prof_mu);
    p.ms += l->prof[i].ms; p.launches += l->prof[i].launches; p.flops += l->prof[i].flops; p.bytes += l->prof[i].bytes;
  }
  if (ms) *ms = p.ms;
  if (launches) *launches = p.launches;
  if (flops) *flops = p.flops;
  if (bytes) *bytes = p.bytes;
  return FW_OK;
}
int32_t fw_synchronize(fw_model* fm) {
  FW_CHECK_ARG(fm, "null model");
  FW_HIP(hipSetDevice(fm->impl.device));
  FW_HIP(hipStreamSynchronize(fm->impl.stream));
  if (fm->impl.dec_stream) FW_HIP(hipStreamSynchronize(fm->impl.dec_stream));
  for (Model* l : fm->impl.xlanes)
    if (l && l->dec_stream) FW_HIP(hipStreamSynchronize(l->dec_stream));
  return FW_OK;
}
int32_t fw_dev_alloc(fw_model* fm, int64_t bytes, void** out_dev) {
  FW_CHECK_ARG(fm && out_dev && bytes >= 0, "bad argument");
  FW_HIP(hipSetDevice(fm->impl.device));
  return dev_alloc(out_dev, (size_t)bytes);
}
int32_t fw_dev_free(fw_model* fm, void* dev) {
  FW_CHECK_ARG(fm, "null model");
  FW_HIP(hipSetDevice(fm->impl.device));
  if (dev) FW_HIP(hipFree(dev));
  return FW_OK;
}
int32_t fw_dev_upload(fw_model* fm, void* dst_dev, const void* src_host, int64_t bytes) {
  FW_CHECK_ARG(fm && dst_dev && src_host && bytes >= 0, "bad argument");
  FW_HIP(hipSetDevice(fm->impl.device));
  FW_HIP(hipMemcpy(dst_dev, src_host, (size_t)bytes, hipMemcpyHostToDevice));
  return FW_OK;
}

static int upload_f16(Model* m, const float* src, size_t n, half_t** dst) {
  int rc = dev_alloc_t(dst, n);
  if (rc) return rc;
  std::vector<uint16_t> tmp(n);
  for (size_t i = 0; i < n; ++i) tmp[i] = f32_to_f16_bits(src[i]);
  FW_HIP(hipMemcpy(*dst, tmp.data(), n * 2, hipMemcpyHostToDevice));
  return FW_OK;
}
static int download_f16(Model* m, const half_t* src, size_t n, float* dst) {
  std::vector<uint16_t> tmp(n);
  FW_HIP(hipStreamSynchronize(m->stream));
  FW_HIP(hipMemcpy(tmp.data(), src, n * 2, hipMemcpyDeviceToHost));
  for (size_t i = 0; i < n; ++i) {
    half_t h;
    memcpy(&h, &tmp[i], 2);
    dst[i] = (float)h;
  }
  return FW_OK;
}

static inline size_t cross_kv_frag_pos(bool vt, int kvp, int mm, int n) {
  const int c = n & 63, r = mm & 31;
  const size_t head = (size_t)(n >> 6) * kvp * 64;
  return vt ? head + ((size_t)((mm >> 5) * 4 + (c >> 4)) * 64 + ((mm >> 3) & 3) * 16 + (c & 15)) * 8 + (mm & 7)
            : head + ((size_t)((mm >> 5) * 4 + 2 * ((r >> 2) & 1) + (c >> 5)) * 64 + ((c >> 3) & 3) * 16 + (((r >> 3) << 2) | (r & 3))) * 8 + (c & 7);
}

static void quant_w_rows_host(const float* W, int N, int K, int8_t* wq, float* ws) {
  for (int n = 0; n < N; ++n) {
    float amax = 0.f;
    for (int k = 0; k < K; ++k) amax = std::max(amax, fabsf(f16_bits_to_f32(f32_to_f16_bits(W[(size_t)n * K + k]))));
    const float sc = amax > 0.f ? 127.0f / amax : 0.f;
    for (int k = 0; k < K; ++k)
      wq[(size_t)n * K + k] = (int8_t)lrintf(f16_bits_to_f32(f32_to_f16_bits(W[(size_t)n * K + k])) * sc);
    ws[n] = amax > 0.f ? amax / 127.0f : 1.0f;
  }
}

int32_t fw_test_gemm(fw_model* fm, const float* A, const float* W, const float* bias, const float* residual,
                     int32_t M, int32_t N, int32_t K, int32_t act_gelu, int32_t use_int8, float* out) {
  FW_CHECK_ARG(fm && A && W && out, "null argument");
  Model* m = &fm->impl;
  std::lock_guard<std::mutex> lk(m->mu);
  FW_HIP(hipSetDevice(m->device));
  half_t *dA = nullptr, *dW = nullptr, *dB = nullptr, *dR = nullptr, *dC = nullptr;
  int rc;
  if ((rc = upload_f16(m, A, (size_t)M * K, &dA))) return rc;
  if ((rc = upload_f16(m, W, (size_t)N * K, &dW))) return rc;
  if (bias && (rc = upload_f16(m, bias, N, &dB))) return rc;
  if (residual && (rc = upload_f16(m, residual, (size_t)M * N, &dR))) return rc;
  if ((rc = dev_alloc_t(&dC, (size_t)M * N))) return rc;
  LinearW L{dW, dB, nullptr, nullptr, nullptr, nullptr, N, K};
  int8_t* dWq = nullptr;
  float* dWs = nullptr;
  if (use_int8) {
    if (m->compute_type != FW_COMPUTE_INT8_FLOAT16 || (int64_t)M * K > (int64_t)m->max_batch * 1500 * 4 * m->cfg.d_model ||
        M > m->max_batch * 1500) {
      set_error("int8 gemm test needs an int8_float16 model and M*K within its quantisation workspace");
      return FW_EINVAL;
    }
    std::vector<int8_t> wq((size_t)N * K);
    std::vector<float> ws(N);
    quant_w_rows_host(W, N, K, wq.data(), ws.data());
    if ((rc = dev_alloc_t(&dWq, wq.size()))) return rc;
    if ((rc = dev_alloc_t(&dWs, ws.size()))) return rc;
    FW_HIP(hipMemcpy(dWq, wq.data(), wq.size(), hipMemcpyHostToDevice));
    FW_HIP(hipMemcpy(dWs, ws.data(), ws.size() * sizeof(float), hipMemcpyHostToDevice));
    L.wq = dWq; L.wscale = dWs;
    if (act_gelu >= 2)
      rc = run_linear_i8(m, L, dA, nullptr, dC, M, 0, nullptr, 0, 0, M, 1, act_gelu - 2, true, 0);
    else
      rc = run_linear_i8(m, L, dA, nullptr, dC, N, 0, dR, N, 0, M, 1, act_gelu, false, 0);
  } else if (act_gelu == 8 || act_gelu == 9) {
    const bool vt = act_gelu == 9;
    if (N % 64 || residual) { set_error("fragment-major gemm test: N %% 64 == 0, no residual"); return FW_EINVAL; }
    const int kvp = (M + 31) / 32 * 32, H = N / 64;
    half_t* dF = nullptr;
    if ((rc = dev_alloc_t(&dF, (size_t)H * kvp * 64))) return rc;
    FW_HIP(hipMemsetAsync(dF, 0, (size_t)H * kvp * 64 * sizeof(half_t), m->stream));
    rc = vt ? run_linear(m, L, dA, K, 0, dF, kvp, 0, nullptr, 0, 0, M, 1, 0, true, kvp)
            : run_linear(m, L, dA, K, 0, dF, N, 0, nullptr, 0, 0, M, 1, 0, false, kvp);
    std::vector<float> hf((size_t)H * kvp * 64);
    if (!rc) rc = download_f16(m, dF, hf.size(), hf.data());
    (void)hipFree(dF);
    if (!rc) {
      for (int mm = 0; mm < kvp && !rc; ++mm)
        for (int n = 0; n < N; ++n) {
          const size_t off = cross_kv_frag_pos(vt, kvp, mm, n);
          if (mm < M) out[(size_t)mm * N + n] = hf[off];
          else if (hf[off] != 0.f) { set_error("fragment-major epilogue wrote the padded key %d", mm); rc = FW_ERUNTIME; break; }
        }
    }
    for (half_t* p : {dA, dW, dB, dR, dC})
      if (p) (void)hipFree(p);
    return rc;
  } else if (act_gelu >= 2) {
    rc = run_linear(m, L, dA, K, 0, dC, M, 0, nullptr, 0, 0, M, 1, act_gelu - 2, true);
  } else {
    rc = run_linear(m, L, dA, K, 0, dC, N, 0, dR, N, 0, M, 1, act_gelu, false);
  }
  if (!rc) rc = download_f16(m, dC, (size_t)M * N, out);
  for (half_t* p : {dA, dW, dB, dR, dC})
    if (p) (void)hipFree(p);
  if (dWq) (void)hipFree(dWq);
  if (dWs) (void)hipFree(dWs);
  return rc;
}

static inline size_t frag_pos(int64_t row, int64_t k, int64_t K, int KE) {
  const int OCT = KE / 4;
  return (size_t)((((row >> 4) * (K / KE) + k / KE) * 64 + ((k / OCT) & 3) * 16 + (row & 15)) * OCT + (k % OCT));
}

int32_t fw_test_dec_linear(fw_model* fm, const float* x, const float* W, const float* bias, const float* ln_g,
                           const float* ln_b, const float* res, int32_t R, int32_t N, int32_t K, int32_t act,
                           int32_t use_int8, float* out, float* out_from_frag) {
  FW_CHECK_ARG(fm && x && W && out && out_from_frag, "null argument");
  FW_CHECK_ARG(R >= 1 && N % 32 == 0 && K % 64 == 0, "need R >= 1, N %% 32 == 0, K %% 64 == 0");
  FW_CHECK_ARG((ln_g == nullptr) == (ln_b == nullptr), "ln_g and ln_b go together");
  Model* m = &fm->impl;
  std::lock_guard<std::mutex> lk(m->mu);
  FW_HIP(hipSetDevice(m->device));
  hipStream_t st = m->stream;
  const int R16 = (R + 15) / 16 * 16;
  auto h = [](float v) { return f16_bits_to_f32(f32_to_f16_bits(v)); };
  std::vector<void*> owned;
  auto up = [&](const void* src, size_t bytes, void** dst) -> int {
    int rc = dev_alloc(dst, bytes);
    if (rc) return rc;
    owned.push_back(*dst);
    FW_HIP(hipMemcpy(*dst, src, bytes, hipMemcpyHostToDevice));
    return FW_OK;
  };
  auto cleanup = [&]() { for (void* p : owned) (void)hipFree(p); };
  int rc = FW_OK;
  half_t *d_res = nullptr, *d_bias = nullptr, *d_out = nullptr, *d_of = nullptr;
  std::vector<uint16_t> tmp;
  if (res) {
    tmp.resize((size_t)R * N);
    for (size_t i = 0; i < tmp.size(); ++i) tmp[i] = f32_to_f16_bits(res[i]);
    if ((rc = up(tmp.data(), tmp.size() * 2, (void**)&d_res))) { cleanup(); return rc; }
  }
  if ((rc = dev_alloc_t(&d_out, (size_t)R * N))) { cleanup(); return rc; }
  owned.push_back(d_out);
  if ((rc = dev_alloc_t(&d_of, (size_t)R16 * N))) { cleanup(); return rc; }
  owned.push_back(d_of);
  FW_HIP(hipMemsetAsync(d_of, 0, (size_t)R16 * N * 2, st));
  if (use_int8 == 1) {
    if (m->compute_type != FW_COMPUTE_INT8_FLOAT16 || ln_g) {
      cleanup();
      set_error("int8 decoder-linear test needs an int8_float16 model and no LayerNorm");
      return FW_EINVAL;
    }
    std::vector<int8_t> wq((size_t)N * K);
    std::vector<float> ws(N);
    for (int n = 0; n < N; ++n) {
      float amax = 0.f;
      for (int k = 0; k < K; ++k) amax = std::max(amax, fabsf(h(W[(size_t)n * K + k])));
      const float sc = amax > 0.f ? 127.0f / amax : 0.f;
      for (int k = 0; k < K; ++k) wq[frag_pos(n, k, K, 64)] = (int8_t)lrintf(h(W[(size_t)n * K + k]) * sc);
      ws[n] = amax > 0.f ? amax / 127.0f : 1.0f;
    }
    int8_t *d_wq = nullptr, *d_xq = nullptr;
    float *d_ws = nullptr, *d_xs = nullptr;
    half_t* d_x = nullptr;
    tmp.resize((size_t)R * K);
    for (size_t i = 0; i < tmp.size(); ++i) tmp[i] = f32_to_f16_bits(x[i]);
    if ((rc = up(wq.data(), wq.size(), (void**)&d_wq)) || (rc = up(ws.data(), ws.size() * 4, (void**)&d_ws)) ||
        (rc = up(tmp.data(), tmp.size() * 2, (void**)&d_x))) { cleanup(); return rc; }
    if (bias) {
      tmp.resize(N);
      for (int n = 0; n < N; ++n) tmp[n] = f32_to_f16_bits(bias[n]);
      if ((rc = up(tmp.data(), (size_t)N * 2, (void**)&d_bias))) { cleanup(); return rc; }
    }
    if ((rc = dev_alloc_t(&d_xq, (size_t)R16 * K))) { cleanup(); return rc; }
    owned.push_back(d_xq);
    if ((rc = dev_alloc_t(&d_xs, (size_t)R16))) { cleanup(); return rc; }
    owned.push_back(d_xs);
    FW_HIP(hipMemsetAsync(d_xq, 0, (size_t)R16 * K, st));
    fwk::launch_quant_rows(st, d_x, K, nullptr, nullptr, d_xq, d_xs, R, K, 1);
    if (fwd::launch_dec_gemm_frag_i8(st, d_xq, d_xs, d_wq, d_ws, d_bias, d_res, N, d_out, N, R, N, K, act) != 0) {
      cleanup();
      set_error("int8 decoder linear: unsupported shape R=%d N=%d K=%d", R, N, K);
      return FW_ERUNTIME;
    }
    rc = download_f16(m, d_out, (size_t)R * N, out);
    if (!rc) memcpy(out_from_frag, out, (size_t)R * N * sizeof(float));
    cleanup();
    return rc;
  }
  std::vector<uint16_t> wf((size_t)N * K), xf((size_t)R16 * K, 0);
  std::vector<float> s1(N, 0.f), cf(N, 0.f);
  for (int n = 0; n < N; ++n) {
    double a1 = 0.0, ac = 0.0;
    for (int k = 0; k < K; ++k) {
      const float wv = h(W[(size_t)n * K + k]);
      const uint16_t wg = ln_g ? f32_to_f16_bits(wv * h(ln_g[k])) : f32_to_f16_bits(wv);
      wf[frag_pos(n, k, K, 32)] = wg;
      a1 += (double)f16_bits_to_f32(wg);
      if (ln_g) ac += (double)wv * (double)h(ln_b[k]);
    }
    if (bias) ac += (double)h(bias[n]);
    s1[n] = (float)a1;
    cf[n] = (float)ac;
  }
  for (int r = 0; r < R; ++r)
    for (int k = 0; k < K; ++k) xf[frag_pos(r, k, K, 32)] = f32_to_f16_bits(x[(size_t)r * K + k]);
  half_t *d_wf = nullptr, *d_xf = nullptr;
  float *d_s1 = nullptr, *d_cf = nullptr;
  if ((rc = up(wf.data(), wf.size() * 2, (void**)&d_wf)) || (rc = up(xf.data(), xf.size() * 2, (void**)&d_xf))) {
    cleanup();
    return rc;
  }
  if (ln_g) {
    if ((rc = up(s1.data(), (size_t)N * 4, (void**)&d_s1)) || (rc = up(cf.data(), (size_t)N * 4, (void**)&d_cf))) {
      cleanup();
      return rc;
    }
  } else if (bias) {
    tmp.resize(N);
    for (int n = 0; n < N; ++n) tmp[n] = f32_to_f16_bits(bias[n]);
    if ((rc = up(tmp.data(), (size_t)N * 2, (void**)&d_bias))) { cleanup(); return rc; }
  }
  const int lr =
      use_int8 >= 10 ? fwd::launch_dec_gemm_big(st, use_int8 - 10, d_xf, d_wf, d_bias, d_s1, d_cf, d_res, N, d_out, N, d_of, R, N, K, act)
      : use_int8 == 5 ? fwd::launch_dec_gemm_skinny(st, d_xf, d_wf, d_bias, d_s1, d_cf, d_res, N, d_out, N, d_of, R, N, K, act)
      : (use_int8 == 6 || use_int8 == 7) ? fwd::launch_dec_gemm_skinny_tiles(st, use_int8 - 5, d_xf, d_wf, d_bias, d_s1, d_cf, d_res, N, d_out, N, d_of, R, N, K, act)
                      : fwd::launch_dec_gemm_frag(st, d_xf, d_wf, d_bias, d_s1, d_cf, d_res, N, d_out, N, d_of, R, N, K, act);
  if (lr != 0) {
    cleanup();
    set_error("decoder linear: unsupported shape R=%d N=%d K=%d", R, N, K);
    return FW_ERUNTIME;
  }
  rc = download_f16(m, d_out, (size_t)R * N, out);
  std::vector<float> of((size_t)R16 * N);
  if (!rc) rc = download_f16(m, d_of, (size_t)R16 * N, of.data());
  if (!rc)
    for (int r = 0; r < R; ++r)
      for (int n = 0; n < N; ++n) out_from_frag[(size_t)r * N + n] = of[frag_pos(r, n, N, 32)];
  cleanup();
  return rc;
}

int32_t fw_dec_big_min_rows(void) { return fwd::dec_big_min_rows(); }
int32_t fw_dec_big_min_rows_of(int32_t role, int32_t compute_type) { return fwd::dec_big_min_rows_of(role, compute_type); }

int32_t fw_test_knob(int32_t id, int32_t value) {
  FW_CHECK_ARG(id == 1 || id == 2 || id == 4 || id == 5 || id == 6 || id == 7, "unknown knob %d", id);
  if (id == 6) { set_cross_kv_layered(value); return FW_OK; }
  if (id == 7) { fwd::set_cross_attn_regs(value); return FW_OK; }
  if (id == 1) fwk::g_gemm_order.store(value);
  else if (id == 5) fwk::g_gemm_vt_stage.store(value);
  else if (id == 2) fwd::set_self_attn_form(value);
  else set_pos_blocks(value);
  return FW_OK;
}

int64_t fw_test_idle_lead_chunks(int64_t queued, int32_t n_queued, int32_t encoding, int64_t want, int32_t max_batch) {
  return idle_lead_chunks(queued, n_queued, encoding, want, max_batch);
}

int32_t fw_test_dec_logits(fw_model* fm, const float* x, int32_t R, float* out) {
  FW_CHECK_ARG(fm && x && out && R >= 1, "bad argument");
  Model* m = &fm->impl;
  std::lock_guard<std::mutex> lk(m->mu);
  FW_HIP(hipSetDevice(m->device));
  hipStream_t st = m->stream;
  const int d = m->cfg.d_model, V = m->cfg.n_vocab, R16 = (R + 15) / 16 * 16;
  const bool i8 = m->compute_type == FW_COMPUTE_INT8_FLOAT16;
  std::vector<uint16_t> xh((size_t)R16 * d, 0);
  for (int r = 0; r < R; ++r)
    for (int k = 0; k < d; ++k)
      xh[i8 ? (size_t)r * d + k : frag_pos(r, k, d, 32)] = f32_to_f16_bits(x[(size_t)r * d + k]);
  half_t* d_x = nullptr;
  int8_t* d_xq = nullptr;
  float *d_xs = nullptr, *d_out = nullptr;
  int rc;
  auto cleanup = [&]() { for (void* p : {(void*)d_x, (void*)d_xq, (void*)d_xs, (void*)d_out}) if (p) (void)hipFree(p); };
  if ((rc = dev_alloc_t(&d_x, xh.size())) || (rc = dev_alloc_t(&d_out, (size_t)R * V))) { cleanup(); return rc; }
  FW_HIP(hipMemcpy(d_x, xh.data(), xh.size() * 2, hipMemcpyHostToDevice));
  int lr;
  if (i8) {
    if ((rc = dev_alloc_t(&d_xq, (size_t)R16 * d)) || (rc = dev_alloc_t(&d_xs, (size_t)R16))) { cleanup(); return rc; }
    FW_HIP(hipMemsetAsync(d_xq, 0, (size_t)R16 * d, st));
    fwk::launch_quant_rows(st, d_x, d, m->dec_ln.g, m->dec_ln.b, d_xq, d_xs, R, d, 1);
    lr = fwd::launch_dec_logits(st, true, d_xq, d_xs, m->logits.wq, m->logits.wscale, nullptr, nullptr, d_out, V, R, V, d);
  } else {
    lr = fwd::launch_dec_logits(st, false, d_x, nullptr, m->logits.w, nullptr, m->logits.s1, m->logits.cf, d_out, V, R, V,
                                d);
  }
  hipError_t he = hipSuccess;
  if (lr == 0) he = hipMemcpyAsync(out, d_out, (size_t)R * V * sizeof(float), hipMemcpyDeviceToHost, st);
  if (he == hipSuccess) he = hipStreamSynchronize(st);
  cleanup();
  if (lr != 0 || he != hipSuccess) {
    set_error("logits projection test failed: %s", lr ? "unsupported shape" : hipGetErrorString(he));
    return FW_ERUNTIME;
  }
  return FW_OK;
}

int32_t fw_bench_dec_linear(fw_model* fm, int32_t R, int32_t N, int32_t K, int32_t lnf, int32_t variant, int32_t iters,
                            float* us_out) {
  FW_CHECK_ARG(fm && us_out && R > 0 && N > 0 && K > 0 && iters > 0, "bad argument");
  Model* m = &fm->impl;
  std::lock_guard<std::mutex> lk(m->mu);
  FW_HIP(hipSetDevice(m->device));
  const size_t wn = (size_t)N * K;
  const int copies = (int)std::max<size_t>(2, ((size_t)640 << 20) / (wn * 2));
  const size_t rp = ((size_t)R + 15) / 16 * 16;
  half_t *dW = nullptr, *dX = nullptr, *dO = nullptr, *dB = nullptr;
  float *dS = nullptr, *dC = nullptr;
  int rc;
  auto cleanup = [&]() { for (void* p : {(void*)dW, (void*)dX, (void*)dO, (void*)dB, (void*)dS, (void*)dC}) if (p) (void)hipFree(p); };
  if ((rc = dev_alloc_t(&dW, wn * copies)) || (rc = dev_alloc_t(&dX, rp * K)) || (rc = dev_alloc_t(&dO, rp * N)) ||
      (rc = dev_alloc_t(&dB, (size_t)N)) || (rc = dev_alloc_t(&dS, (size_t)N)) || (rc = dev_alloc_t(&dC, (size_t)N))) {
    cleanup();
    return rc;
  }
  {
    std::vector<uint16_t> h(std::max(wn, rp * (size_t)K));
    uint32_t sd = 2463534242u;
    for (auto& v : h) { sd = sd * 1664525u + 1013904223u; v = f32_to_f16_bits(((int)(sd >> 16) % 2001 - 1000) * 1e-3f); }
    for (int c = 0; c < copies; ++c) FW_HIP(hipMemcpy(dW + (size_t)c * wn, h.data(), wn * 2, hipMemcpyHostToDevice));
    FW_HIP(hipMemcpy(dX, h.data(), rp * K * 2, hipMemcpyHostToDevice));
  }
  FW_HIP(hipMemset(dB, 0, (size_t)N * 2));
  FW_HIP(hipMemset(dS, 0, (size_t)N * 4));
  FW_HIP(hipMemset(dC, 0, (size_t)N * 4));
  hipEvent_t e0, e1;
  FW_HIP(hipEventCreate(&e0));
  FW_HIP(hipEventCreate(&e1));
  hipStream_t st = m->stream;
  int lr = 0;
  for (int i = 0; i < 4 && lr == 0; ++i)
    lr = fwd::launch_dec_gemm_frag_variant(st, variant, lnf != 0, dX, dW + (size_t)(i % copies) * wn, dB, dS, dC, dO, R, N, K);
  FW_HIP(hipEventRecord(e0, st));
  for (int i = 0; i < iters && lr == 0; ++i)
    lr = fwd::launch_dec_gemm_frag_variant(st, variant, lnf != 0, dX, dW + (size_t)(i % copies) * wn, dB, dS, dC, dO, R, N, K);
  FW_HIP(hipEventRecord(e1, st));
  hipError_t he = hipEventSynchronize(e1);
  float ms = 0.f;
  if (he == hipSuccess) he = hipEventElapsedTime(&ms, e0, e1);
  (void)hipEventDestroy(e0);
  (void)hipEventDestroy(e1);
  cleanup();
  if (lr != 0) { set_error("fw_bench_dec_linear: unsupported shape / variant"); return FW_EINVAL; }
  if (he != hipSuccess) { set_error("fw_bench_dec_linear: %s", hipGetErrorString(he)); return FW_ENODEV; }
  *us_out = ms * 1000.f / (float)iters;
  return FW_OK;
}

int32_t fw_bench_gemm(fw_model* fm, int32_t M, int32_t N, int32_t K, int32_t batch, int32_t a_pad, int32_t w_pad,
                      int32_t trans, int32_t iters, float* ms_out) {
  FW_CHECK_ARG(fm && ms_out && M > 0 && N > 0 && K > 0 && batch > 0 && iters > 0, "bad argument");
  Model* m = &fm->impl;
  std::lock_guard<std::mutex> lk(m->mu);
  FW_HIP(hipSetDevice(m->device));
  const bool i8 = m->compute_type == FW_COMPUTE_INT8_FLOAT16;
  const int64_t lda = K + a_pad, ldw = K + w_pad;
  const size_t es = i8 ? 1 : 2;
  const int64_t ldct = (M + 63) / 64 * 64;
  const size_t na = (size_t)batch * M * lda, nw = (size_t)N * ldw,
               nc = trans ? (size_t)batch * N * ldct : (size_t)batch * M * N;
  void *dA = nullptr, *dW = nullptr;
  half_t* dC = nullptr;
  float *dsa = nullptr, *dsw = nullptr;
  int rc;
  auto cleanup = [&]() { for (void* p : {dA, dW, (void*)dC, (void*)dsa, (void*)dsw}) if (p) (void)hipFree(p); };
  if ((rc = dev_alloc(&dA, na * es)) || (rc = dev_alloc(&dW, nw * es)) || (rc = dev_alloc_t(&dC, nc))) { cleanup(); return rc; }
  {
    std::vector<uint16_t> h(std::max(na, nw));
    uint32_t st = 12345u;
    for (auto& v : h) { st = st * 1664525u + 1013904223u; v = f32_to_f16_bits(((int)(st >> 16) % 2001 - 1000) * 1e-3f); }
    FW_HIP(hipMemcpy(dA, h.data(), na * es, hipMemcpyHostToDevice));
    FW_HIP(hipMemcpy(dW, h.data(), nw * es, hipMemcpyHostToDevice));
  }
  if (i8) {
    if ((rc = dev_alloc_t(&dsa, (size_t)batch * M)) || (rc = dev_alloc_t(&dsw, (size_t)N))) { cleanup(); return rc; }
    FW_HIP(hipMemset(dsa, 0, (size_t)batch * M * 4));
    FW_HIP(hipMemset(dsw, 0, (size_t)N * 4));
  }
  fwk::GemmParams p;
  memset(&p, 0, sizeof(p));
  p.A = (const half_t*)dA; p.lda = lda; p.a_bstride = (int64_t)M * lda;
  p.W = (const half_t*)dW; p.ldw = ldw;
  p.C = dC; p.ldc = trans ? ldct : N; p.c_bstride = trans ? (int64_t)N * ldct : (int64_t)M * N;
  p.M = M; p.N = N; p.K = K;
  p.a_scale = dsa; p.as_bstride = M; p.w_scale = dsw;
  hipEvent_t e0, e1;
  FW_HIP(hipEventCreate(&e0));
  FW_HIP(hipEventCreate(&e1));
  int lr = fwk::launch_gemm(m->stream, p, batch, trans != 0);
  FW_HIP(hipEventRecord(e0, m->stream));
  for (int i = 0; i < iters && lr == 0; ++i) lr = fwk::launch_gemm(m->stream, p, batch, trans != 0);
  FW_HIP(hipEventRecord(e1, m->stream));
  hipError_t he = hipEventSynchronize(e1);
  float ms = 0.f;
  if (he == hipSuccess) he = hipEventElapsedTime(&ms, e0, e1);
  (void)hipEventDestroy(e0);
  (void)hipEventDestroy(e1);
  cleanup();
// ... 250 lines not shown
  const int64_t a_last = (int64_t)(batch - 1) * a_bstride + (int64_t)(M - 1) * lda + (K - 1);
  FW_CHECK_ARG(a_last < a_elems, "the launch reads A[%lld], a_elems = %lld", (long long)a_last, (long long)a_elems);
  if (res) {
    const int64_t r_last = (int64_t)(batch - 1) * r_bstride + (int64_t)(M - 1) * ldr + (N - 1);
    FW_CHECK_ARG(r_last < r_elems, "the launch reads res[%lld], r_elems = %lld", (long long)r_last, (long long)r_elems);
  }
  const int64_t chunk_last = head_rows > 0 ? (int64_t)(N / 64 - 1) * head_rows * 64 + (int64_t)((M - 1) / 32 + 1) * 2048 - 1
                             : trans       ? (int64_t)(N - 1) * ldc + (M - 1)
                                           : (int64_t)(M - 1) * ldc + (N - 1);
  const int64_t c_last = c_off + (int64_t)(n_layers - 1) * c_lstride + (int64_t)(batch - 1) * c_bstride + chunk_last;
  FW_CHECK_ARG(c_last < c_elems, "the launch writes C[%lld], c_elems = %lld", (long long)c_last, (long long)c_elems);

  Model* m = &fm->impl;
  std::lock_guard<std::mutex> lk(m->mu);
  if (use_int8) {
    const int64_t T = m->cfg.n_audio_ctx;
    if (m->compute_type != FW_COMPUTE_INT8_FLOAT16 || (int64_t)batch * M * K > (int64_t)m->max_batch * T * 4 * m->cfg.d_model ||
        (int64_t)batch * M > (int64_t)m->max_batch * T || (ln_g && K > 1536)) {
      set_error("int8 gemm test needs an int8_float16 model, batch*M*K within its quantisation workspace, K <= 1536 with LayerNorm");
      return FW_EINVAL;
    }
  }
  FW_HIP(hipSetDevice(m->device));
  std::vector<void*> owned;
  auto cleanup = [&]() { for (void* p : owned) (void)hipFree(p); };
  auto up16 = [&](const float* src, size_t n, half_t** dst) -> int {
    int rc = upload_f16(m, src, n, dst);
    if (*dst) owned.push_back(*dst);
    return rc;
  };
  half_t *dA = nullptr, *dW = nullptr, *dB = nullptr, *dR = nullptr, *dC = nullptr, *dG = nullptr, *dLb = nullptr;
  const size_t nw = (size_t)n_layers * N * K;
  int rc;
  if ((rc = up16(A, (size_t)a_elems, &dA)) || (rc = up16(W, nw, &dW)) || (bias && (rc = up16(bias, (size_t)n_layers * N, &dB))) ||
      (res && (rc = up16(res, (size_t)r_elems, &dR))) || (rc = up16(C, (size_t)c_elems, &dC)) ||
      (ln_g && ((rc = up16(ln_g, K, &dG)) || (rc = up16(ln_b, K, &dLb))))) { cleanup(); return rc; }
  LinearW L{dW, dB, nullptr, nullptr, nullptr, nullptr, N, K};
  if (use_int8) {
    std::vector<int8_t> wq(nw);
    std::vector<float> ws(N);
    quant_w_rows_host(W, N, K, wq.data(), ws.data());
    int8_t* dWq = nullptr;
    float* dWs = nullptr;
    if ((rc = dev_alloc_t(&dWq, wq.size()))) { cleanup(); return rc; }
    owned.push_back(dWq);
    if ((rc = dev_alloc_t(&dWs, ws.size()))) { cleanup(); return rc; }
    owned.push_back(dWs);
    if (hipMemcpy(dWq, wq.data(), wq.size(), hipMemcpyHostToDevice) != hipSuccess ||
        hipMemcpy(dWs, ws.data(), ws.size() * sizeof(float), hipMemcpyHostToDevice) != hipSuccess) {
      cleanup();
      set_error("fw_test_gemm_ex: upload failed");
      return FW_ENODEV;
    }
    L.wq = dWq; L.wscale = dWs;
    LNW ln{dG, dLb};
    rc = run_linear_i8(m, L, dA, ln_g ? &ln : nullptr, dC + c_off, ldc, c_bstride, dR, ldr, r_bstride, M, batch, act,
                       trans != 0, head_rows);
  } else if (n_layers > 1) {
    rc = run_linear_layers(m, L, n_layers, (int64_t)N * K, bias ? N : 0, dA, lda, a_bstride, dC + c_off, ldc, c_bstride,
                           c_lstride, M, batch, trans != 0, head_rows, nullptr);
  } else {
    rc = run_linear(m, L, dA, lda, a_bstride, dC + c_off, ldc, c_bstride, dR, ldr, r_bstride, M, batch, act, trans != 0,
                    head_rows, nullptr);
  }
  if (!rc) rc = download_f16(m, dC, (size_t)c_elems, C);
  cleanup();
  return rc;
}

int32_t fw_test_attention(fw_model* fm, const float* q, const float* k, const float* v, int32_t B, int32_t H,
                          int32_t T, float* out) {
  FW_CHECK_ARG(fm && q && k && v && out, "null argument");
  Model* m = &fm->impl;
  std::lock_guard<std::mutex> lk(m->mu);
  FW_HIP(hipSetDevice(m->device));
  const int d = H * 64, tp = (T + 63) / 64 * 64;
  const size_t n = (size_t)B * T * d;
  half_t *dq = nullptr, *dk = nullptr, *dvt = nullptr, *dout = nullptr;
  int rc;
  if ((rc = upload_f16(m, q, n, &dq))) return rc;
  if ((rc = upload_f16(m, k, n, &dk))) return rc;
  std::vector<float> vt((size_t)B * d * tp, 0.f);
  for (int b = 0; b < B; ++b)
    for (int t = 0; t < T; ++t)
      for (int c = 0; c < d; ++c) vt[((size_t)b * d + c) * tp + t] = v[((size_t)b * T + t) * d + c];
  if ((rc = upload_f16(m, vt.data(), vt.size(), &dvt))) return rc;
  if ((rc = dev_alloc_t(&dout, n))) return rc;
  fwk::launch_attn_enc(m->stream, dq, dk, d, (int64_t)T * d, dvt, tp, (int64_t)d * tp, dout, d, (int64_t)T * d, B, H,
                       T);
  rc = download_f16(m, dout, n, out);
  for (half_t* p : {dq, dk, dvt, dout})
    if (p) (void)hipFree(p);
  return rc;
}

int32_t fw_bench_attention(fw_model* fm, int32_t B, int32_t H, int32_t T, int32_t variant, int32_t iters, float* ms_out) {
  FW_CHECK_ARG(fm && ms_out && B > 0 && H > 0 && T > 0 && iters > 0, "bad argument");
  Model* m = &fm->impl;
  std::lock_guard<std::mutex> lk(m->mu);
  FW_HIP(hipSetDevice(m->device));
  const int d = H * 64, tp = (T + 63) / 64 * 64;
  const size_t nqk = (size_t)B * T * 2 * d, nvt = (size_t)B * d * tp, no = (size_t)B * T * d;
  half_t *dqk = nullptr, *dvt = nullptr, *dout = nullptr;
  int rc;
  auto cleanup = [&]() { for (half_t* p : {dqk, dvt, dout}) if (p) (void)hipFree(p); };
  if ((rc = dev_alloc_t(&dqk, nqk)) || (rc = dev_alloc_t(&dvt, nvt)) || (rc = dev_alloc_t(&dout, no))) { cleanup(); return rc; }
  {
    std::vector<uint16_t> h(std::max(nqk, nvt));
    uint32_t sd = 777u;
    for (auto& v : h) { sd = sd * 1664525u + 1013904223u; v = f32_to_f16_bits(((int)(sd >> 16) % 2001 - 1000) * 2e-3f); }
    FW_HIP(hipMemcpy(dqk, h.data(), nqk * 2, hipMemcpyHostToDevice));
    FW_HIP(hipMemcpy(dvt, h.data(), nvt * 2, hipMemcpyHostToDevice));
  }
  hipEvent_t e0, e1;
  FW_HIP(hipEventCreate(&e0));
  FW_HIP(hipEventCreate(&e1));
  auto go = [&]() {
    fwk::launch_attn_enc(m->stream, dqk, dqk + d, 2 * d, (int64_t)T * 2 * d, dvt, tp, (int64_t)d * tp, dout, d, (int64_t)T * d, B,
                         H, T, variant);
  };
  go();
  FW_HIP(hipEventRecord(e0, m->stream));
  for (int i = 0; i < iters; ++i) go();
  FW_HIP(hipEventRecord(e1, m->stream));
  hipError_t he = hipEventSynchronize(e1);
  float ms = 0.f;
  if (he == hipSuccess) he = hipEventElapsedTime(&ms, e0, e1);
  (void)hipEventDestroy(e0);
  (void)hipEventDestroy(e1);
  cleanup();
  if (he != hipSuccess) { set_error("attention bench failed: %s", hipGetErrorString(he)); return FW_ERUNTIME; }
  *ms_out = ms / (float)iters;
  return FW_OK;
}

extern "C++" {
namespace {
struct DevBufs {
  std::vector<void*> p;
  template <typename T>
  int alloc(T** dst, size_t n) {
    int rc = dev_alloc_t(dst, n);
    if (!rc) p.push_back(*dst);
    return rc;
  }
  ~DevBufs() { for (void* q : p) (void)hipFree(q); }
};
int upload_f16_to(const float* src, size_t n, half_t* dst) {
  std::vector<uint16_t> tmp(n);
  for (size_t i = 0; i < n; ++i) tmp[i] = f32_to_f16_bits(src[i]);
  FW_HIP(hipMemcpy(dst, tmp.data(), n * 2, hipMemcpyHostToDevice));
  return FW_OK;
}
}
}

int32_t fw_test_dec_self_attn(fw_model* fm, const float* qkv, float* kcache, float* vcache, const uint8_t* kvidx,
                              int32_t n_chunks, int32_t kmul, int32_t Kbeam, int32_t H, int32_t n_ctx, int32_t cache_ctx,
                              int32_t pos_fixed, int32_t P, int32_t step, int32_t blk_n, int32_t frag, float* out) {
  FW_CHECK_ARG(fm && qkv && kcache && vcache && kvidx && out, "null argument");
  FW_CHECK_ARG(n_chunks >= 1 && H >= 1 && kmul >= 1 && kmul <= 16 && Kbeam >= 1 && Kbeam <= 255, "bad geometry");
  FW_CHECK_ARG(n_ctx >= 1 && n_ctx <= 448 && cache_ctx >= 1 && cache_ctx <= n_ctx, "need 1 <= cache_ctx <= n_ctx <= 448");
  FW_CHECK_ARG(blk_n >= 0 && (blk_n == 0 ? kmul <= Kbeam : (kmul == blk_n && pos_fixed >= 0)),
               "blk_n = 0: kmul <= Kbeam; blk_n > 0: kmul == blk_n and pos_fixed >= 0");
  const int pos0 = pos_fixed >= 0 ? pos_fixed : P - 1 + step;
  const int pos_last = pos0 + (blk_n > 0 ? blk_n - 1 : 0);
  FW_CHECK_ARG(pos0 >= 0 && pos_last < cache_ctx, "positions %d..%d outside the cache (%d)", pos0, pos_last, cache_ctx);
  const int d = H * 64, R = n_chunks * kmul, R16 = (R + 15) / 16 * 16, R_total = n_chunks * Kbeam;
  FW_CHECK_ARG(blk_n == 0 || fwd::self_attn_block_ok(n_ctx, cache_ctx, d, R_total), "position blocks need n_ctx %% 4 == 0");
  const size_t n_tab = (size_t)2 * R_total * n_ctx, n_cache = (size_t)R_total * H * cache_ctx * 64;
  for (size_t i = 0; i < n_tab; ++i)
    FW_CHECK_ARG(kvidx[i] < Kbeam, "kvidx[%zu] = %d is not a beam of %d", i, (int)kvidx[i], Kbeam);
  Model* m = &fm->impl;
  std::lock_guard<std::mutex> lk(m->mu);
  FW_HIP(hipSetDevice(m->device));
  DevBufs db;
  half_t *d_qkv, *d_kc, *d_vc, *d_out;
  uint8_t* d_idx;
  int* d_step;
  int rc;
  if ((rc = db.alloc(&d_qkv, (size_t)R * 3 * d)) || (rc = db.alloc(&d_kc, n_cache)) || (rc = db.alloc(&d_vc, n_cache)) ||
      (rc = db.alloc(&d_out, (size_t)R16 * d)) || (rc = db.alloc(&d_idx, n_tab)) || (rc = db.alloc(&d_step, 1)))
    return rc;
  if ((rc = upload_f16_to(qkv, (size_t)R * 3 * d, d_qkv)) || (rc = upload_f16_to(kcache, n_cache, d_kc)) ||
      (rc = upload_f16_to(vcache, n_cache, d_vc)))
    return rc;
  FW_HIP(hipMemcpy(d_idx, kvidx, n_tab, hipMemcpyHostToDevice));
  FW_HIP(hipMemcpy(d_step, &step, sizeof(int), hipMemcpyHostToDevice));
  FW_HIP(hipMemsetAsync(d_out, 0, (size_t)R16 * d * 2, m->stream));
  fwd::launch_self_attn(m->stream, d_qkv, d, d_kc, d_vc, n_ctx, cache_ctx, H, d_idx, Kbeam, kmul, d_out, R, d_step,
                        pos_fixed, P, R_total, frag ? 1 : 0, blk_n);
  FW_HIP(hipGetLastError());
  if ((rc = download_f16(m, d_kc, n_cache, kcache)) || (rc = download_f16(m, d_vc, n_cache, vcache))) return rc;
  if (!frag) return download_f16(m, d_out, (size_t)R * d, out);
  std::vector<float> of((size_t)R16 * d);
  if ((rc = download_f16(m, d_out, of.size(), of.data()))) return rc;
  for (int r = 0; r < R; ++r)
    for (int n = 0; n < d; ++n) out[(size_t)r * d + n] = of[frag_pos(r, n, d, 32)];
  return FW_OK;
}

int32_t fw_test_dec_cross_attn(fw_model* fm, const float* q, const float* k, const float* v, int32_t n_enc, int32_t T,
                               int32_t H, int32_t B, int32_t kmul, int32_t kv_div, const int32_t* slot_map,
                               const int32_t* done, int32_t frag, float k_pad, float* out) {
  FW_CHECK_ARG(fm && q && k && v && slot_map && out, "null argument");
  FW_CHECK_ARG(n_enc >= 1 && T >= 1 && H >= 1 && B >= 1 && kmul >= 1 && kmul <= 16 && kv_div >= 1, "bad geometry");
  const int n_map = (B + kv_div - 1) / kv_div;
  for (int i = 0; i < n_map; ++i)
    FW_CHECK_ARG(slot_map[i] >= 0 && slot_map[i] < n_enc, "slot_map[%d] = %d outside [0, %d)", i, slot_map[i], n_enc);
  const int d = H * 64, kvp = (T + 31) / 32 * 32, R = B * kmul, R16 = (R + 15) / 16 * 16;
  const size_t blk = (size_t)d * kvp;
  std::vector<float> kf((size_t)n_enc * blk), vf((size_t)n_enc * blk, 0.f);
  for (int e = 0; e < n_enc; ++e)
    for (int t = 0; t < kvp; ++t)
      for (int n = 0; n < d; ++n) {
        const size_t src = ((size_t)e * T + t) * d + n;
        kf[e * blk + cross_kv_frag_pos(false, kvp, t, n)] = t < T ? k[src] : k_pad;
        if (t < T) vf[e * blk + cross_kv_frag_pos(true, kvp, t, n)] = v[src];
      }
  std::vector<float> of((size_t)R16 * d, 0.f);
  if (frag)
    for (int r = 0; r < R; ++r)
      for (int n = 0; n < d; ++n) of[frag_pos(r, n, d, 32)] = out[(size_t)r * d + n];
  Model* m = &fm->impl;
  std::lock_guard<std::mutex> lk(m->mu);
  FW_HIP(hipSetDevice(m->device));
  DevBufs db;
  half_t *d_q, *d_k, *d_vt, *d_out;
  int *d_map, *d_done = nullptr;
  int rc;
  if ((rc = db.alloc(&d_q, (size_t)R * d)) || (rc = db.alloc(&d_k, kf.size())) || (rc = db.alloc(&d_vt, vf.size())) ||
      (rc = db.alloc(&d_out, (size_t)R16 * d)) || (rc = db.alloc(&d_map, (size_t)n_map)) || (done && (rc = db.alloc(&d_done, (size_t)B))))
    return rc;
  if ((rc = upload_f16_to(q, (size_t)R * d, d_q)) || (rc = upload_f16_to(kf.data(), kf.size(), d_k)) ||
      (rc = upload_f16_to(vf.data(), vf.size(), d_vt)) || (rc = upload_f16_to(frag ? of.data() : out, frag ? of.size() : (size_t)R * d, d_out)))
    return rc;
  FW_HIP(hipMemcpy(d_map, slot_map, (size_t)n_map * sizeof(int), hipMemcpyHostToDevice));
  if (done) FW_HIP(hipMemcpy(d_done, done, (size_t)B * sizeof(int), hipMemcpyHostToDevice));
  fwd::launch_cross_attn(m->stream, d_q, d, d_k, d_vt, T, kvp, kmul, d_out, B, H, d_done, kv_div, frag ? 1 : 0, d_map);
  FW_HIP(hipGetLastError());
  if (!frag) return download_f16(m, d_out, (size_t)R * d, out);
  if ((rc = download_f16(m, d_out, of.size(), of.data()))) return rc;
  for (int r = 0; r < R; ++r)
    for (int n = 0; n < d; ++n) out[(size_t)r * d + n] = of[frag_pos(r, n, d, 32)];
  return FW_OK;
}

int32_t fw_test_dec_cross_probs(fw_model* fm, const float* q, const float* k, int32_t B, int32_t T, int32_t H,
                                const int32_t* heads, int32_t n_sel, int32_t n_tok, int32_t tok_idx, int32_t blk_n,
                                float* probs) {
  FW_CHECK_ARG(fm && q && k && heads && probs, "null argument");
  const int blk = blk_n > 0 ? blk_n : 1;
  FW_CHECK_ARG(B >= 1 && T >= 1 && H >= 1 && n_sel >= 1 && blk_n >= 0 && blk <= 16, "bad geometry");
  FW_CHECK_ARG(tok_idx >= 0 && tok_idx + blk <= n_tok, "tokens %d..%d outside [0, %d)", tok_idx, tok_idx + blk - 1, n_tok);
  for (int i = 0; i < n_sel; ++i) FW_CHECK_ARG(heads[i] >= 0 && heads[i] < H, "heads[%d] = %d outside [0, %d)", i, heads[i], H);
  const int d = H * 64, kvp = (T + 31) / 32 * 32;
  const size_t blkk = (size_t)d * kvp, n_probs = (size_t)B * n_sel * n_tok * T;
  std::vector<float> kf((size_t)B * blkk, 0.f);
  for (int b = 0; b < B; ++b)
    for (int t = 0; t < T; ++t)
      for (int n = 0; n < d; ++n) kf[b * blkk + cross_kv_frag_pos(false, kvp, t, n)] = k[((size_t)b * T + t) * d + n];
  Model* m = &fm->impl;
  std::lock_guard<std::mutex> lk(m->mu);
  FW_HIP(hipSetDevice(m->device));
  DevBufs db;
  half_t *d_q, *d_k;
  int* d_heads;
  float* d_p;
  int rc;
  if ((rc = db.alloc(&d_q, (size_t)B * blk * d)) || (rc = db.alloc(&d_k, kf.size())) || (rc = db.alloc(&d_heads, (size_t)n_sel)) ||
      (rc = db.alloc(&d_p, n_probs)))
    return rc;
  if ((rc = upload_f16_to(q, (size_t)B * blk * d, d_q)) || (rc = upload_f16_to(kf.data(), kf.size(), d_k))) return rc;
  FW_HIP(hipMemcpy(d_heads, heads, (size_t)n_sel * sizeof(int), hipMemcpyHostToDevice));
  FW_HIP(hipMemcpy(d_p, probs, n_probs * sizeof(float), hipMemcpyHostToDevice));
  fwd::launch_cross_probs(m->stream, d_q, d, d_k, T, kvp, d_heads, n_sel, n_sel, d_p, n_tok, tok_idx, B, blk_n);
  FW_HIP(hipGetLastError());
  FW_HIP(hipStreamSynchronize(m->stream));
  FW_HIP(hipMemcpy(probs, d_p, n_probs * sizeof(float), hipMemcpyDeviceToHost));
  return FW_OK;
}

int32_t fw_test_dec_softmax_pick(fw_model* fm, const float* logits, int32_t rows, int32_t V, int32_t row_mul,
                                 const int32_t* target, int32_t nospeech, float* out) {
  FW_CHECK_ARG(fm && logits && target && out, "null argument");
  FW_CHECK_ARG(rows >= 1 && V >= 1 && row_mul >= 1, "bad geometry");
  FW_CHECK_ARG(!nospeech || (target[0] >= 0 && target[0] < V), "no-speech id %d outside [0, %d)", target[0], V);
  Model* m = &fm->impl;
  std::lock_guard<std::mutex> lk(m->mu);
  FW_HIP(hipSetDevice(m->device));
  DevBufs db;
  const size_t n_lg = (size_t)rows * row_mul * V;
  float *d_lg, *d_out;
  int* d_t;
  int rc;
  if ((rc = db.alloc(&d_lg, n_lg)) || (rc = db.alloc(&d_out, (size_t)rows)) || (rc = db.alloc(&d_t, (size_t)rows))) return rc;
  FW_HIP(hipMemcpy(d_lg, logits, n_lg * sizeof(float), hipMemcpyHostToDevice));
  FW_HIP(hipMemcpy(d_t, target, (size_t)(nospeech ? 1 : rows) * sizeof(int), hipMemcpyHostToDevice));
  if (nospeech) fwd::launch_nospeech(m->stream, d_lg, V, row_mul, target[0], d_out, rows);
  else fwd::launch_token_prob(m->stream, d_lg, V, d_t, d_out, 1, 0, rows, row_mul);
  FW_HIP(hipGetLastError());
  FW_HIP(hipStreamSynchronize(m->stream));
  FW_HIP(hipMemcpy(out, d_out, (size_t)rows * sizeof(float), hipMemcpyDeviceToHost));
  return FW_OK;
}

}
```

Measured before the change: 3236.

## Fuse cross-attention query projection with layernorm into the cross-attention kernel

Adds a fused variant of the decoder cross-attention kernel in which each block computes its own query rows: LayerNorm statistics, a matmul against the folded cross-Q weights and the epilogue, with a reduction through shared memory. This replaces the separate cross-Q GEMM launch and the round trip of the query tensor through global memory. It is enabled by default when the row count is at least 800 and the layer is not int8, unfused or producing alignment probabilities. The cost is that the Q weight slice for each head is re-read by every batch-chunk block instead of once, and the kernel gains extra synchronisation. Also adds a test entry point, a micro-benchmark and small LN helper refactors.

```diff
diff --git a/faster_whisper_amd/_lib.py b/faster_whisper_amd/_lib.py
--- a/faster_whisper_amd/_lib.py
+++ b/faster_whisper_amd/_lib.py
@@ -73,7 +73,7 @@
     "fw_prof_enable", "fw_prof_reset", "fw_prof_count", "fw_prof_name", "fw_prof_get", "fw_synchronize",
     "fw_dev_alloc", "fw_dev_free", "fw_dev_upload",
     "fw_test_gemm", "fw_test_layernorm", "fw_test_attention", "fw_test_dec_linear", "fw_test_dec_logits", "fw_test_logits_rules",
-    "fw_test_dec_self_attn", "fw_test_dec_cross_attn", "fw_test_dec_cross_probs", "fw_test_dec_softmax_pick", "fw_bench_gemm", "fw_bench_dec_linear", "fw_bench_attention",
+    "fw_test_dec_self_attn", "fw_test_dec_cross_attn", "fw_test_dec_cross_attn_fused", "fw_bench_dec_cross_q", "fw_test_dec_cross_probs", "fw_test_dec_softmax_pick", "fw_bench_gemm", "fw_bench_dec_linear", "fw_bench_attention",
     "fw_bench_gemm_epi", "fw_bench_dec_linear_epi",
     "fw_test_gemm_ex", "fw_test_cross_kv_frag_index", "fw_test_quant_rows", "fw_test_layernorm_frag",
     "fw_vad_create", "fw_vad_forward", "fw_vad_free", "fw_vad_forward_dev", "fw_vad_forward_audio_dev",
@@ -167,6 +167,10 @@
         lib.fw_test_dec_cross_attn.argtypes = [vp, vp, vp, vp, i32, i32, i32, i32, i32, i32, vp, vp, i32, C.c_float, vp]
         lib.fw_test_dec_cross_probs.argtypes = [vp, vp, vp, i32, i32, i32, vp, i32, i32, i32, i32, vp]
         lib.fw_test_dec_softmax_pick.argtypes = [vp, vp, i32, i32, i32, vp, i32, vp]
+    if hasattr(lib, "fw_test_dec_cross_attn_fused"):
+        lib.fw_test_dec_cross_attn_fused.argtypes = [vp, vp, vp, vp, vp, vp, vp, vp, i32, i32, i32, i32, i32, i32, vp, vp,
+                                                     i32, C.c_float, i32, vp, vp]
+        lib.fw_bench_dec_cross_q.argtypes = [vp, i32, i32, i32, i32, i32, i32, f32p]
     lib.fw_bench_attention.argtypes = [vp, i32, i32, i32, i32, i32, f32p]
     lib.fw_bench_gemm.argtypes = [vp, i32, i32, i32, i32, i32, i32, i32, i32, f32p]
     lib.fw_bench_dec_linear.argtypes = [vp, i32, i32, i32, i32, i32, i32, f32p]
diff --git a/faster_whisper_amd/csrc/dec_kernels.h b/faster_whisper_amd/csrc/dec_kernels.h
--- a/faster_whisper_amd/csrc/dec_kernels.h
+++ b/faster_whisper_amd/csrc/dec_kernels.h
@@ -35,6 +35,11 @@
 void bump_kernel_forms_epoch();
 void launch_cross_attn(hipStream_t st, const half_t* qx, int d, const half_t* ck, const half_t* cvt, int T, int kvp,
                        int kmul, half_t* out, int B, int H, const int* done, int kv_div, int frag, const int* slot_map);
+int launch_cross_attn_fused(hipStream_t st, const half_t* xf, const half_t* Wf, const float* s1, const float* cf, int d,
+                            const half_t* ck, const half_t* cvt, int T, int kvp, int kmul, half_t* out, int B, int H,
+                            const int* done, int kv_div, int frag, const int* slot_map);
+bool cross_q_fused_for(int rows, int d);
+void set_cross_q_fused(int v);
 int dec_big_min_rows();
 int dec_big_min_rows_of(int role, int compute_type);
 int launch_dec_gemm_frag(hipStream_t st, const half_t* xf, const half_t* Wf, const half_t* bias, const float* s1,
diff --git a/faster_whisper_amd/csrc/dec_kernels.hip b/faster_whisper_amd/csrc/dec_kernels.hip
--- a/faster_whisper_amd/csrc/dec_kernels.hip
+++ b/faster_whisper_amd/csrc/dec_kernels.hip
@@ -7,6 +7,7 @@
 namespace fwd {
 static std::atomic<int> g_self_attn_form{0};
 static std::atomic<int> g_forms_epoch{0};
+static std::atomic<int> g_cross_q_fused{-1};
 static std::atomic<int> g_cross_regs{0};
 }
 
@@ -33,6 +34,20 @@
   }
 }
 
+static __device__ __forceinline__ void dec_ln_accum(const half8_t x, float& rs, float& rq) {
+  const half2_t one2 = {(half_t)1.f, (half_t)1.f};
+#pragma unroll
+  for (int e = 0; e < 4; ++e) {
+    const half2_t h2 = {x[2 * e], x[2 * e + 1]};
+    rs = __builtin_amdgcn_fdot2(h2, one2, rs, false);
+    rq = __builtin_amdgcn_fdot2(h2, h2, rq, false);
+  }
+}
+static __device__ __forceinline__ float dec_ln_quad_sum(float v) {
+  v += __shfl_xor(v, 16, 64);
+  v += __shfl_xor(v, 32, 64);
+  return v;
+}
 static __device__ __forceinline__ void dec_ln_stats(float sa, float sb, int K, float& mu, float& rstd) {
 #pragma clang fp contract(off)
   const float kf = (float)K;
@@ -183,15 +198,7 @@
 #pragma unroll
             for (int b = 0; b < NT; ++b)
               acc[a][b] = __builtin_amdgcn_mfma_f32_16x16x32_f16(wv[b][j], xv[a][j], acc[a][b], 0, 0, 0);
-            if (LNF) {
-              const half2_t one2 = {(half_t)1.f, (half_t)1.f};
-#pragma unroll
-              for (int e = 0; e < 4; ++e) {
-                const half2_t h2 = {xv[a][j][2 * e], xv[a][j][2 * e + 1]};
-                rs[a] = __builtin_amdgcn_fdot2(h2, one2, rs[a], false);
-                rq[a] = __builtin_amdgcn_fdot2(h2, h2, rq[a], false);
-              }
-            }
+            if (LNF) dec_ln_accum(xv[a][j], rs[a], rq[a]);
           }
         }
       }
@@ -212,9 +219,7 @@
 #pragma unroll
   for (int a = 0; a < RT; ++a) {
     if (LNF) {
-      float sa = rs[a], sb = rq[a];
-      sa += __shfl_xor(sa, 16, 64); sa += __shfl_xor(sa, 32, 64);
-      sb += __shfl_xor(sb, 16, 64); sb += __shfl_xor(sb, 32, 64);
+      const float sa = dec_ln_quad_sum(rs[a]), sb = dec_ln_quad_sum(rq[a]);
       if (g == 0) { red_s[wave][a][i][0] = sa; red_s[wave][a][i][1] = sb; }
     }
 #pragma unroll
@@ -359,16 +364,9 @@
 #pragma unroll
     for (int ks = 0; ks < KC; ++ks) {
       if (LNF) {
-        const half2_t one2 = {(half_t)1.f, (half_t)1.f};
         const half8_t xs0 = wn ? xv[ks][2] : xv[ks][0], xs1 = wn ? xv[ks][3] : xv[ks][1];
-#pragma unroll
-        for (int e = 0; e < 4; ++e) {
-          const half2_t h0 = {xs0[2 * e], xs0[2 * e + 1]}, h1 = {xs1[2 * e], xs1[2 * e + 1]};
-          rs[0] = __builtin_amdgcn_fdot2(h0, one2, rs[0], false);
-          rq[0] = __builtin_amdgcn_fdot2(h0, h0, rq[0], false);
-          rs[1] = __builtin_amdgcn_fdot2(h1, one2, rs[1], false);
-          rq[1] = __builtin_amdgcn_fdot2(h1, h1, rq[1], false);
-        }
+        dec_ln_accum(xs0, rs[0], rq[0]);
+        dec_ln_accum(xs1, rs[1], rq[1]);
       }
 #pragma unroll
       for (int b = 0; b < FB; ++b) {
@@ -383,10 +381,7 @@
     if (LNF) {
 #pragma unroll
       for (int aa = 0; aa < 2; ++aa) {
-        float pa = rs[aa], pb = rq[aa];
-        pa += __shfl_xor(pa, 16, 64); pa += __shfl_xor(pa, 32, 64);
-        pb += __shfl_xor(pb, 16, 64); pb += __shfl_xor(pb, 32, 64);
-        sal[aa] += pa; sbl[aa] += pb;
+        sal[aa] += dec_ln_quad_sum(rs[aa]); sbl[aa] += dec_ln_quad_sum(rq[aa]);
         rs[aa] = 0.f; rq[aa] = 0.f;
       }
     }
@@ -1044,15 +1039,20 @@
   }
 }
 
-template <int CA_WAVES, bool NTL, int MINW = 1>
+template <int CA_WAVES, bool NTL, int MINW = 1, bool FQ = false>
 __global__ __launch_bounds__(CA_WAVES * 64, MINW) void dec_cross_attn_kernel(const half_t* __restrict__ qx, int d,
                                                              const half_t* __restrict__ ck,
                                                              const half_t* __restrict__ cvt, int T, int kvp,
                                                              int kmul, half_t* __restrict__ out,
                                                              const int* __restrict__ done, int kv_div, int frag,
-                                                             const int* __restrict__ slot_map) {
+                                                             const int* __restrict__ slot_map,
+                                                             const half_t* __restrict__ xf = nullptr,
+                                                             const half_t* __restrict__ Wf = nullptr,
+                                                             const float* __restrict__ s1 = nullptr,
+                                                             const float* __restrict__ cf = nullptr) {
+  static_assert(!FQ || CA_WAVES == 8, "the fused projection spreads 4 column tiles x 4 K slices over 8 waves");
   __shared__ float sm[CA_WAVES][16], sl[CA_WAVES][16];
-  __shared__ float so[CA_WAVES][16][65];
+  __shared__ __attribute__((aligned(16))) float so[CA_WAVES][16][65];
   const int h = blockIdx.x, c = blockIdx.y;
   if (done && done[c]) return;
   const int tid = threadIdx.x, lane = tid & 63, wave = tid >> 6;
@@ -1061,12 +1061,11 @@
   const half_t* kbase = ck + ((size_t)ce * (d >> 6) + h) * kvp * 64 + lane * 8;
   const half_t* vbase = cvt + ((size_t)ce * (d >> 6) + h) * kvp * 64 + lane * 8;
   half8_t qf[2];
-  {
+  auto read_q = [&](auto qp) {
     if (j < kmul) {
-      const half_t* qp = qx + (size_t)(c * kmul + j) * d + h * 64 + g * 8;
 #pragma unroll
       for (int s = 0; s < 2; ++s) {
-        half8_t v = *reinterpret_cast<const half8_t*>(qp + s * 32);
+        half8_t v = *reinterpret_cast<const half8_t*>(qp + g * 8 + s * 32);
 #pragma unroll
         for (int e = 0; e < 8; ++e) v[e] = v[e] * (half_t)0.125f;
         qf[s] = v;
@@ -1075,12 +1074,8 @@
       qf[0] = half8_t{0, 0, 0, 0, 0, 0, 0, 0};
       qf[1] = qf[0];
     }
-  }
-  floatx4 o[4];
-#pragma unroll
-  for (int dt = 0; dt < 4; ++dt) o[dt] = floatx4{0, 0, 0, 0};
-  float m_run = -1.0e30f, l_run = 0.f;
-  const float LOG2E = 1.4426950408889634f;
+  };
+  if constexpr (!FQ) read_q(qx + (size_t)(c * kmul + j) * d + h * 64);
   const int ngroups = (T + 31) >> 5;
   auto load_kv = [&](int gi, half8_t (&kf)[4], half8_t (&vf)[4]) {
     const half_t* kp = kbase + (size_t)gi * 2048;
@@ -1096,6 +1091,81 @@
   };
   half8_t kcur[4], vcur[4], knxt[4], vnxt[4];
   if (wave < ngroups) load_kv(wave, kcur, vcur);
+  if constexpr (FQ) {
+    constexpr int QT_LD = 72;
+    __shared__ __attribute__((aligned(16))) half_t qt[16 * QT_LD];
+    __builtin_amdgcn_sched_barrier(0);
+    float* part = &so[0][0][0];
+    float* pst = part + 4 * 4 * 64 * 4;
+    const int KS = d >> 5, per = KS >> 2;
+    const int wu = __builtin_amdgcn_readfirstlane(wave);
+    const int slice = wu & 3, cb = (wu >> 2) * 2;
+    const int r0 = c * kmul;
+    constexpr int CHQ = 5;
+    for (int rt = r0 >> 4; rt <= (r0 + kmul - 1) >> 4; ++rt) {
+      const half8_t* xp = reinterpret_cast<const half8_t*>(xf) + ((size_t)rt * KS + slice * per) * 64;
+      const half8_t* wp0 = reinterpret_cast<const half8_t*>(Wf) + ((size_t)(h * 4 + cb) * KS + slice * per) * 64;
+      const half8_t* wp1 = wp0 + (size_t)KS * 64;
+      floatx4 acc0 = {0, 0, 0, 0}, acc1 = {0, 0, 0, 0};
+      float rs = 0.f, rq = 0.f;
+      auto ksteps = [&](auto nq, int k0) {
+        constexpr int NQ = decltype(nq)::value;
+        half8_t xv[NQ], wv0[NQ], wv1[NQ];
+#pragma unroll
+        for (int q = 0; q < NQ; ++q) {
+          xv[q] = xp[(k0 + q) * 64 + lane];
+          wv0[q] = wp0[(k0 + q) * 64 + lane];
+          wv1[q] = wp1[(k0 + q) * 64 + lane];
+        }
+#pragma unroll
+        for (int q = 0; q < NQ; ++q) {
+          acc0 = __builtin_amdgcn_mfma_f32_16x16x32_f16(wv0[q], xv[q], acc0, 0, 0, 0);
+          acc1 = __builtin_amdgcn_mfma_f32_16x16x32_f16(wv1[q], xv[q], acc1, 0, 0, 0);
+          dec_ln_accum(xv[q], rs, rq);
+        }
+      };
+      int k0 = 0;
+      for (; k0 + CHQ <= per; k0 += CHQ) ksteps(std::integral_constant<int, CHQ>{}, k0);
+      switch (per - k0) {
+        case 4: ksteps(std::integral_constant<int, 4>{}, k0); break;
+        case 3: ksteps(std::integral_constant<int, 3>{}, k0); break;
+        case 2: ksteps(std::integral_constant<int, 2>{}, k0); break;
+        case 1: ksteps(std::integral_constant<int, 1>{}, k0); break;
+        default: break;
+      }
+      int ncol = h * 64 + slice * 16 + 4 * g;
+      asm volatile("" : "+v"(ncol));
+      const DecColConsts colk = dec_col_consts<true>(s1, cf, nullptr, ncol);
+      rs = dec_ln_quad_sum(rs); rq = dec_ln_quad_sum(rq);
+      if (wu < 4 && g == 0) { pst[(slice * 16 + j) * 2] = rs; pst[(slice * 16 + j) * 2 + 1] = rq; }
+      *reinterpret_cast<floatx4*>(part + ((slice * 4 + cb) * 64 + lane) * 4) = acc0;
+      *reinterpret_cast<floatx4*>(part + ((slice * 4 + cb + 1) * 64 + lane) * 4) = acc1;
+      __syncthreads();
+      if (wu < 4) {
+        float v[4] = {0.f, 0.f, 0.f, 0.f}, sa = 0.f, sb = 0.f;
+#pragma unroll
+        for (int w = 0; w < 4; ++w) {
+          const floatx4 p4 = *reinterpret_cast<const floatx4*>(part + ((w * 4 + wu) * 64 + lane) * 4);
+#pragma unroll
+          for (int e = 0; e < 4; ++e) v[e] += p4[e];
+          sa += pst[(w * 16 + j) * 2]; sb += pst[(w * 16 + j) * 2 + 1];
+        }
+        float mu, rstd;
+        dec_ln_stats(sa, sb, d, mu, rstd);
+        const floatx4 v4 = {v[0], v[1], v[2], v[3]};
+        const half4_t o4 = dec_epilogue4<true>(v4, mu, rstd, colk.a4, colk.c4, colk.b4, false, false, colk.b4, 0);
+        const int jq = rt * 16 + j - r0;
+        if (jq >= 0 && jq < kmul) *reinterpret_cast<half4_t*>(qt + jq * QT_LD + wu * 16 + 4 * g) = o4;
+      }
+      __syncthreads();
+    }
+    read_q(qt + j * QT_LD);
+  }
+  floatx4 o[4];
+#pragma unroll
+  for (int dt = 0; dt < 4; ++dt) o[dt] = floatx4{0, 0, 0, 0};
+  float m_run = -1.0e30f, l_run = 0.f;
+  const float LOG2E = 1.4426950408889634f;
   for (int gi = wave; gi < ngroups; gi += CA_WAVES) {
     const int base = gi * 32;
     const bool has_next = (gi + CA_WAVES) < ngroups;
@@ -1847,6 +1917,31 @@
 }
 void set_cross_attn_regs(int cap) { g_cross_regs.store(cap); g_forms_epoch.fetch_add(1); }
 
+struct CrossQRule { int from, upto; };
+static const CrossQRule CROSS_Q_FUSED_ROWS = {800, 1 << 30};
+bool cross_q_fused_for(int rows, int d) {
+  if ((d >> 5) % 4 != 0 || d % 64 != 0) return false;
+  int mode = g_cross_q_fused.load(std::memory_order_relaxed);
+  if (mode < 0) {
+    const char* e = getenv("FWAMD_CROSS_Q_FUSED");
+    mode = e ? atoi(e) : 1;
+    if (mode < 0 || mode > 2) mode = 1;
+    g_cross_q_fused.store(mode);
+  }
+  if (mode != 1) return mode == 2;
+  return rows >= CROSS_Q_FUSED_ROWS.from && rows <= CROSS_Q_FUSED_ROWS.upto;
+}
+void set_cross_q_fused(int v) { g_cross_q_fused.store(v == 1 ? 0 : (v == 2 ? 2 : -1)); g_forms_epoch.fetch_add(1); }
+
+int launch_cross_attn_fused(hipStream_t st, const half_t* xf, const half_t* Wf, const float* s1, const float* cf, int d,
+                            const half_t* ck, const half_t* cvt, int T, int kvp, int kmul, half_t* out, int B, int H,
+                            const int* done, int kv_div, int frag, const int* slot_map) {
+  if ((d >> 5) % 4 != 0 || d != H * 64 || !s1 || !cf || kmul < 1 || kmul > 16) return -1;
+  dec_cross_attn_kernel<8, true, 1, true><<<dim3(H, B), 512, 0, st>>>(nullptr, d, ck, cvt, T, kvp, kmul, out, done, kv_div,
+                                                                        frag, slot_map, xf, Wf, s1, cf);
+  return 0;
+}
+
 void launch_nospeech(hipStream_t st, const float* logits, int V, int row_mul, int no_speech_id, float* out, int B) {
   dec_nospeech_kernel<<<B, 1024, 0, st>>>(logits, V, row_mul, no_speech_id, out);
 }
diff --git a/faster_whisper_amd/csrc/decoder.hip b/faster_whisper_amd/csrc/decoder.hip
--- a/faster_whisper_amd/csrc/decoder.hip
+++ b/faster_whisper_amd/csrc/decoder.hip
@@ -439,18 +439,21 @@
       fwd::launch_self_attn(st, g->qkv, d, kc, vc, NT, gp.ctx, H, g->kvidx2, gp.K, s.kmul, frag ? g->att_frag : g->att, rows,
                             g->d_step, s.pos_fixed, s.P, gp.R, frag, s.blk_n);
     }
+    const bool layer_probs = s.probs && s.sel_layer_off[l + 1] > s.sel_layer_off[l];
+    const bool fuse_q = !i8 && !unf && !layer_probs && s.kmul <= 16 && fwd::cross_q_fused_for(rows, d);
     {
-      ProfScope ps(m, PF_DEC_GEMM_DXD, 2.0 * rows * 2.0 * d * d, 2.0 * 2.0 * d * d, st);
+      const double n_lin = fuse_q ? 1.0 : 2.0;
+      ProfScope ps(m, PF_DEC_GEMM_DXD, 2.0 * rows * n_lin * d * d, 2.0 * n_lin * d * d, st);
       if (i8) {
         DG(lin_q(g->att, nullptr, L.out, g->x, g->x, 0));
         DG(lin_q(g->x, &L.ln2, L.cq, nullptr, g->qc, 0));
       } else {
         DG(lin_f(g->att_frag, L.out, g->x, g->x, g->x_frag, 0));
         if (unf) DG(lin_u(L.ln2, L.cq_p, g->qc, nullptr, 0));
-        else DG(lin_f(g->x_frag, L.cq, nullptr, g->qc, nullptr, 0));
+        else if (!fuse_q) DG(lin_f(g->x_frag, L.cq, nullptr, g->qc, nullptr, 0));
       }
     }
-    if (s.probs && s.sel_layer_off[l + 1] > s.sel_layer_off[l]) {
+    if (layer_probs) {
       ProfScope ps(m, PF_DEC_MISC, 0, 0, st);
       const int off = s.sel_layer_off[l], n = s.sel_layer_off[l + 1] - off;
       fwd::launch_cross_probs(st, g->qc, d, ck + (size_t)s.kv_slot0 * d * kvp, T, kvp, s.sel_heads_dev + off, n, s.n_sel_total,
@@ -458,8 +461,12 @@
     }
     {
       ProfScope ps(m, PF_DEC_CROSS_ATTN, 4.0 * rows * (double)T * d, 4.0 * (s.B / gp.kv_div) * (double)T * d, st);
-      fwd::launch_cross_attn(st, g->qc, d, ck, cvt, T, kvp, s.kmul, frag ? g->att_frag : g->att, s.B, H, s.done,
-                             gp.kv_div, frag, g->slot_map);
+      if (fuse_q)
+        DG(fwd::launch_cross_attn_fused(st, g->x_frag, L.cq.w, L.cq.s1, L.cq.cf, d, ck, cvt, T, kvp, s.kmul, g->att_frag, s.B, H,
+                                        s.done, gp.kv_div, 1, g->slot_map));
+      else
+        fwd::launch_cross_attn(st, g->qc, d, ck, cvt, T, kvp, s.kmul, frag ? g->att_frag : g->att, s.B, H, s.done,
+                               gp.kv_div, frag, g->slot_map);
     }
     {
       ProfScope ps(m, PF_DEC_GEMM_DXD, 2.0 * rows * 1.0 * d * d, 2.0 * 1.0 * d * d, st);
diff --git a/faster_whisper_amd/csrc/engine.hip b/faster_whisper_amd/csrc/engine.hip
--- a/faster_whisper_amd/csrc/engine.hip
+++ b/faster_whisper_amd/csrc/engine.hip
@@ -1695,6 +1695,25 @@
   return (size_t)((((row >> 4) * (K / KE) + k / KE) * 64 + ((k / OCT) & 3) * 16 + (row & 15)) * OCT + (k % OCT));
 }
 
+static void fold_linear_host(const float* W, const float* bias, const float* ln_g, const float* ln_b, int N, int K,
+                             std::vector<uint16_t>& wf, std::vector<float>& s1, std::vector<float>& cf) {
+  auto h = [](float v) { return f16_bits_to_f32(f32_to_f16_bits(v)); };
+  wf.assign((size_t)N * K, 0); s1.assign(N, 0.f); cf.assign(N, 0.f);
+  for (int n = 0; n < N; ++n) {
+    double a1 = 0.0, ac = 0.0;
+    for (int k = 0; k < K; ++k) {
+      const float wv = h(W[(size_t)n * K + k]);
+      const uint16_t wg = ln_g ? f32_to_f16_bits(wv * h(ln_g[k])) : f32_to_f16_bits(wv);
+      wf[frag_pos(n, k, K, 32)] = wg;
+      a1 += (double)f16_bits_to_f32(wg);
+      if (ln_g) ac += (double)wv * (double)h(ln_b[k]);
+    }
+    if (bias) ac += (double)h(bias[n]);
+    s1[n] = (float)a1;
+    cf[n] = (float)ac;
+  }
+}
+
 int32_t fw_test_dec_linear(fw_model* fm, const float* x, const float* W, const float* bias, const float* ln_g,
                            const float* ln_b, const float* res, int32_t R, int32_t N, int32_t K, int32_t act,
                            int32_t use_int8, float* out, float* out_from_frag) {
@@ -1772,21 +1791,9 @@
     cleanup();
     return rc;
   }
-  std::vector<uint16_t> wf((size_t)N * K), xf((size_t)R16 * K, 0);
-  std::vector<float> s1(N, 0.f), cf(N, 0.f);
-  for (int n = 0; n < N; ++n) {
-    double a1 = 0.0, ac = 0.0;
-    for (int k = 0; k < K; ++k) {
-      const float wv = h(W[(size_t)n * K + k]);
-      const uint16_t wg = ln_g ? f32_to_f16_bits(wv * h(ln_g[k])) : f32_to_f16_bits(wv);
-      wf[frag_pos(n, k, K, 32)] = wg;
-      a1 += (double)f16_bits_to_f32(wg);
-      if (ln_g) ac += (double)wv * (double)h(ln_b[k]);
-    }
-    if (bias) ac += (double)h(bias[n]);
-    s1[n] = (float)a1;
-    cf[n] = (float)ac;
-  }
+  std::vector<uint16_t> wf, xf((size_t)R16 * K, 0);
+  std::vector<float> s1, cf;
+  fold_linear_host(W, bias, ln_g, ln_b, N, K, wf, s1, cf);
   for (int r = 0; r < R; ++r)
     for (int k = 0; k < K; ++k) xf[frag_pos(r, k, K, 32)] = f32_to_f16_bits(x[(size_t)r * K + k]);
   half_t *d_wf = nullptr, *d_xf = nullptr;
@@ -1829,8 +1836,9 @@
 int32_t fw_dec_big_min_rows_of(int32_t role, int32_t compute_type) { return fwd::dec_big_min_rows_of(role, compute_type); }
 
 int32_t fw_test_knob(int32_t id, int32_t value) {
-  FW_CHECK_ARG(id == 1 || id == 2 || id == 4 || id == 5 || id == 6 || id == 7, "unknown knob %d", id);
+  FW_CHECK_ARG(id == 1 || id == 2 || id == 4 || id == 5 || id == 6 || id == 7 || id == 8, "unknown knob %d", id);
   if (id == 6) { set_cross_kv_layered(value); return FW_OK; }
+  if (id == 8) { fwd::set_cross_q_fused(value); return FW_OK; }
   if (id == 7) { fwd::set_cross_attn_regs(value); return FW_OK; }
   if (id == 1) fwk::g_gemm_order.store(value);
   else if (id == 5) fwk::g_gemm_vt_stage.store(value);
@@ -2387,6 +2395,19 @@
   FW_HIP(hipMemcpy(dst, tmp.data(), n * 2, hipMemcpyHostToDevice));
   return FW_OK;
 }
+void cross_pool_host(const float* k, const float* v, int n_enc, int T, int d, float k_pad, std::vector<float>& kf,
+                     std::vector<float>& vf) {
+  const int kvp = (T + 31) / 32 * 32;
+  const size_t blk = (size_t)d * kvp;
+  kf.assign((size_t)n_enc * blk, 0.f); vf.assign((size_t)n_enc * blk, 0.f);
+  for (int e = 0; e < n_enc; ++e)
+    for (int t = 0; t < kvp; ++t)
+      for (int n = 0; n < d; ++n) {
+        const size_t src = ((size_t)e * T + t) * d + n;
+        kf[e * blk + cross_kv_frag_pos(false, kvp, t, n)] = t < T ? k[src] : k_pad;
+        if (t < T) vf[e * blk + cross_kv_frag_pos(true, kvp, t, n)] = v[src];
+      }
+}
 }
 }
 
@@ -2444,15 +2465,8 @@
   for (int i = 0; i < n_map; ++i)
     FW_CHECK_ARG(slot_map[i] >= 0 && slot_map[i] < n_enc, "slot_map[%d] = %d outside [0, %d)", i, slot_map[i], n_enc);
   const int d = H * 64, kvp = (T + 31) / 32 * 32, R = B * kmul, R16 = (R + 15) / 16 * 16;
-  const size_t blk = (size_t)d * kvp;
-  std::vector<float> kf((size_t)n_enc * blk), vf((size_t)n_enc * blk, 0.f);
-  for (int e = 0; e < n_enc; ++e)
-    for (int t = 0; t < kvp; ++t)
-      for (int n = 0; n < d; ++n) {
-        const size_t src = ((size_t)e * T + t) * d + n;
-        kf[e * blk + cross_kv_frag_pos(false, kvp, t, n)] = t < T ? k[src] : k_pad;
-        if (t < T) vf[e * blk + cross_kv_frag_pos(true, kvp, t, n)] = v[src];
-      }
+  std::vector<float> kf, vf;
+  cross_pool_host(k, v, n_enc, T, d, k_pad, kf, vf);
   std::vector<float> of((size_t)R16 * d, 0.f);
   if (frag)
     for (int r = 0; r < R; ++r)
@@ -2481,6 +2495,135 @@
   return FW_OK;
 }
 
+int32_t fw_test_dec_cross_attn_fused(fw_model* fm, const float* x, const float* ln_g, const float* ln_b, const float* W,
+                                     const float* bias, const float* k, const float* v, int32_t n_enc, int32_t T, int32_t H,
+                                     int32_t B, int32_t kmul, int32_t kv_div, const int32_t* slot_map, const int32_t* done,
+                                     int32_t frag, float k_pad, int32_t two_launches, float* out, float* q_out) {
+  FW_CHECK_ARG(fm && x && ln_g && ln_b && W && k && v && slot_map && out, "null argument");
+  FW_CHECK_ARG(!two_launches || q_out, "the two-launch path returns its q");
+  FW_CHECK_ARG(n_enc >= 1 && T >= 1 && H >= 1 && B >= 1 && kmul >= 1 && kmul <= 16 && kv_div >= 1, "bad geometry");
+  const int n_map = (B + kv_div - 1) / kv_div;
+  for (int i = 0; i < n_map; ++i)
+    FW_CHECK_ARG(slot_map[i] >= 0 && slot_map[i] < n_enc, "slot_map[%d] = %d outside [0, %d)", i, slot_map[i], n_enc);
+  const int d = H * 64, kvp = (T + 31) / 32 * 32, R = B * kmul, R16 = (R + 15) / 16 * 16;
+  std::vector<float> kf, vf;
+  cross_pool_host(k, v, n_enc, T, d, k_pad, kf, vf);
+  std::vector<uint16_t> wf, xf((size_t)R16 * d, 0);
+  std::vector<float> s1, cf;
+  fold_linear_host(W, bias, ln_g, ln_b, d, d, wf, s1, cf);
+  for (int r = 0; r < R; ++r)
+    for (int kk = 0; kk < d; ++kk) xf[frag_pos(r, kk, d, 32)] = f32_to_f16_bits(x[(size_t)r * d + kk]);
+  std::vector<float> of((size_t)R16 * d, 0.f);
+  if (frag)
+    for (int r = 0; r < R; ++r)
+      for (int n = 0; n < d; ++n) of[frag_pos(r, n, d, 32)] = out[(size_t)r * d + n];
+  Model* m = &fm->impl;
+  std::lock_guard<std::mutex> lk(m->mu);
+  FW_HIP(hipSetDevice(m->device));
+  DevBufs db;
+  half_t *d_x, *d_w, *d_q, *d_k, *d_vt, *d_out;
+  float *d_s1, *d_cf;
+  int *d_map, *d_done = nullptr;
+  int rc;
+  if ((rc = db.alloc(&d_x, xf.size())) || (rc = db.alloc(&d_w, wf.size())) || (rc = db.alloc(&d_s1, (size_t)d)) ||
+      (rc = db.alloc(&d_cf, (size_t)d)) || (rc = db.alloc(&d_q, (size_t)R * d)) || (rc = db.alloc(&d_k, kf.size())) ||
+      (rc = db.alloc(&d_vt, vf.size())) || (rc = db.alloc(&d_out, (size_t)R16 * d)) || (rc = db.alloc(&d_map, (size_t)n_map)) ||
+      (done && (rc = db.alloc(&d_done, (size_t)B))))
+    return rc;
+  FW_HIP(hipMemcpy(d_x, xf.data(), xf.size() * 2, hipMemcpyHostToDevice));
+  FW_HIP(hipMemcpy(d_w, wf.data(), wf.size() * 2, hipMemcpyHostToDevice));
+  FW_HIP(hipMemcpy(d_s1, s1.data(), (size_t)d * 4, hipMemcpyHostToDevice));
+  FW_HIP(hipMemcpy(d_cf, cf.data(), (size_t)d * 4, hipMemcpyHostToDevice));
+  if ((rc = upload_f16_to(kf.data(), kf.size(), d_k)) || (rc = upload_f16_to(vf.data(), vf.size(), d_vt)) ||
+      (rc = upload_f16_to(frag ? of.data() : out, frag ? of.size() : (size_t)R * d, d_out)))
+    return rc;
+  FW_HIP(hipMemcpy(d_map, slot_map, (size_t)n_map * sizeof(int), hipMemcpyHostToDevice));
+  if (done) FW_HIP(hipMemcpy(d_done, done, (size_t)B * sizeof(int), hipMemcpyHostToDevice));
+  hipStream_t st = m->stream;
+  int lr;
+  if (two_launches) {
+    lr = fwd::launch_dec_gemm_frag(st, d_x, d_w, nullptr, d_s1, d_cf, nullptr, d, d_q, d, nullptr, R, d, d, 0);
+    if (lr == 0) fwd::launch_cross_attn(st, d_q, d, d_k, d_vt, T, kvp, kmul, d_out, B, H, d_done, kv_div, frag ? 1 : 0, d_map);
+  } else {
+    lr = fwd::launch_cross_attn_fused(st, d_x, d_w, d_s1, d_cf, d, d_k, d_vt, T, kvp, kmul, d_out, B, H, d_done, kv_div,
+                                      frag ? 1 : 0, d_map);
+  }
+  if (lr != 0) { set_error("fused cross-attention: unsupported shape d=%d", d); return FW_ERUNTIME; }
+  FW_HIP(hipGetLastError());
+  if (two_launches && (rc = download_f16(m, d_q, (size_t)R * d, q_out))) return rc;
+  if (!frag) return download_f16(m, d_out, (size_t)R * d, out);
+  if ((rc = download_f16(m, d_out, of.size(), of.data()))) return rc;
+  for (int r = 0; r < R; ++r)
+    for (int n = 0; n < d; ++n) out[(size_t)r * d + n] = of[frag_pos(r, n, d, 32)];
+  return FW_OK;
+}
+
+int32_t fw_bench_dec_cross_q(fw_model* fm, int32_t H, int32_t T, int32_t B, int32_t kmul, int32_t fused, int32_t iters,
+                             float* us_out) {
+  FW_CHECK_ARG(fm && us_out && H >= 1 && T >= 1 && B >= 1 && kmul >= 1 && kmul <= 16 && iters > 0, "bad argument");
+  const int d = H * 64, kvp = (T + 31) / 32 * 32, R = B * kmul, R16 = (R + 15) / 16 * 16;
+  FW_CHECK_ARG((d / 32) % 4 == 0, "d / 32 must be a multiple of 4");
+  Model* m = &fm->impl;
+  std::lock_guard<std::mutex> lk(m->mu);
+  FW_HIP(hipSetDevice(m->device));
+  const size_t blk = (size_t)B * d * kvp, wn = (size_t)d * d;
+  const int copies = (int)std::max<size_t>(2, ((size_t)640 << 20) / (2 * blk * 2) + 1);
+  const int wcopies = (int)std::max<size_t>(2, ((size_t)640 << 20) / (wn * 2));
+  DevBufs db;
+  half_t *d_x, *d_w, *d_q, *d_k, *d_vt, *d_out;
+  float *d_s1, *d_cf;
+  int* d_map;
+  int rc;
+  if ((rc = db.alloc(&d_x, (size_t)R16 * d)) || (rc = db.alloc(&d_w, wn * wcopies)) || (rc = db.alloc(&d_s1, (size_t)d)) ||
+      (rc = db.alloc(&d_cf, (size_t)d)) || (rc = db.alloc(&d_q, (size_t)R16 * d)) || (rc = db.alloc(&d_k, blk * copies)) ||
+      (rc = db.alloc(&d_vt, blk * copies)) || (rc = db.alloc(&d_out, (size_t)R16 * d)) || (rc = db.alloc(&d_map, (size_t)B)))
+    return rc;
+  {
+    std::vector<uint16_t> h;
+    if ((rc = bench_fill(d_w, wn, h, 2463534242u)) || (rc = bench_fill(d_x, (size_t)R16 * d, h, 88172645u)) ||
+        (rc = bench_fill(d_k, blk, h, 362436069u)) || (rc = bench_fill(d_vt, blk, h, 521288629u)))
+      return rc;
+    for (int c = 1; c < wcopies; ++c) FW_HIP(hipMemcpy(d_w + (size_t)c * wn, d_w, wn * 2, hipMemcpyDeviceToDevice));
+    for (int c = 1; c < copies; ++c) {
+      FW_HIP(hipMemcpy(d_k + (size_t)c * blk, d_k, blk * 2, hipMemcpyDeviceToDevice));
+      FW_HIP(hipMemcpy(d_vt + (size_t)c * blk, d_vt, blk * 2, hipMemcpyDeviceToDevice));
+    }
+    std::vector<int> map(B);
+    for (int c = 0; c < B; ++c) map[c] = c;
+    FW_HIP(hipMemcpy(d_map, map.data(), (size_t)B * sizeof(int), hipMemcpyHostToDevice));
+  }
+  FW_HIP(hipMemset(d_s1, 0, (size_t)d * 4));
+  FW_HIP(hipMemset(d_cf, 0, (size_t)d * 4));
+  hipStream_t st = m->stream;
+  auto go = [&](int i) -> int {
+    const half_t* w = d_w + (size_t)(i % wcopies) * wn;
+    const half_t* kk = d_k + (size_t)(i % copies) * blk;
+    const half_t* vv = d_vt + (size_t)(i % copies) * blk;
+    if (fused)
+      return fwd::launch_cross_attn_fused(st, d_x, w, d_s1, d_cf, d, kk, vv, T, kvp, kmul, d_out, B, H, nullptr, 1, 1, d_map);
+    const int lr = fwd::launch_dec_gemm_frag(st, d_x, w, nullptr, d_s1, d_cf, nullptr, d, d_q, d, nullptr, R, d, d, 0);
+    if (lr == 0) fwd::launch_cross_attn(st, d_q, d, kk, vv, T, kvp, kmul, d_out, B, H, nullptr, 1, 1, d_map);
+    return lr;
+  };
+  hipEvent_t e0, e1;
+  FW_HIP(hipEventCreate(&e0));
+  FW_HIP(hipEventCreate(&e1));
+  int lr = 0;
+  for (int i = 0; i < 4 && lr == 0; ++i) lr = go(i);
+  FW_HIP(hipEventRecord(e0, st));
+  for (int i = 0; i < iters && lr == 0; ++i) lr = go(i);
+  FW_HIP(hipEventRecord(e1, st));
+  hipError_t he = hipEventSynchronize(e1);
+  float ms = 0.f;
+  if (he == hipSuccess) he = hipEventElapsedTime(&ms, e0, e1);
+  (void)hipEventDestroy(e0);
+  (void)hipEventDestroy(e1);
+  if (lr != 0) { set_error("fw_bench_dec_cross_q: unsupported shape"); return FW_EINVAL; }
+  if (he != hipSuccess) { set_error("fw_bench_dec_cross_q: %s", hipGetErrorString(he)); return FW_ENODEV; }
+  *us_out = ms * 1000.f / (float)iters;
+  return FW_OK;
+}
+
 int32_t fw_test_dec_cross_probs(fw_model* fm, const float* q, const float* k, int32_t B, int32_t T, int32_t H,
                                 const int32_t* heads, int32_t n_sel, int32_t n_tok, int32_t tok_idx, int32_t blk_n,
                                 float* probs) {
diff --git a/profiles/cross_q_bench.py b/profiles/cross_q_bench.py
--- /dev/null
+++ b/profiles/cross_q_bench.py
@@ -0,0 +1,34 @@
+import argparse, ctypes as C, json, os, sys
+sys.path.insert(0, os.path.dirname(os.path.dirname(os.path.abspath(__file__))))
+
+
+def main():
+    ap = argparse.ArgumentParser()
+    ap.add_argument("--model", default="large-v3")
+    ap.add_argument("--chunks", default="16,160,256")
+    ap.add_argument("--kmul", type=int, default=5)
+    ap.add_argument("--rounds", type=int, default=5)
+    ap.add_argument("--iters", type=int, default=200)
+    a = ap.parse_args()
+    from faster_whisper_amd import Whisper, get_config, synthetic_weights, _lib
+    cfg = get_config("micro")
+    big = get_config(a.model)
+    m = Whisper("synthetic:micro", device="cuda", files={"config": cfg, "weights": synthetic_weights(cfg, seed=1)},
+                compute_type="float16", max_batch_size=2, max_beam_size=2)
+    lib = _lib.load()
+    h = m._replicas[0].handle
+    H, T = big.n_heads, big.n_audio_ctx
+    for B in [int(x) for x in a.chunks.split(",")]:
+        us = {0: [], 1: []}
+        for _ in range(a.rounds):
+            for fused in (0, 1):
+                v = C.c_float()
+                _lib.check(lib.fw_bench_dec_cross_q(h, H, T, B, a.kmul, fused, a.iters, C.byref(v)))
+                us[fused].append(round(v.value, 2))
+        rec = dict(model=a.model, H=H, T=T, chunks=B, kmul=a.kmul, rows=B * a.kmul, two_launches_us=us[0], fused_us=us[1],
+                   two_min=min(us[0]), fused_min=min(us[1]), ratio=round(min(us[1]) / min(us[0]), 4))
+        print(json.dumps(rec), flush=True)
+
+
+if __name__ == "__main__":
+    main()
```

Measured after the change: 3225. No clear change (-0.3%).
